# tc-mb/llama.cpp-omni

Measured on AMD Instinct MI355X. Metric: llama-bench tg128 tok/s (decode, batch 1), Qwen3-8B Q4_K_M, higher is better.
Workload: dtype q4_K/q6_K weights x q8_K activations (int8 dot, f32 accumulate); 1 GPU; Qwen3-8B Q4_K_M text-only decode, batch=1 per GPU, 1xMI355X (mul_mat_vec_q path); n_layer=36, n_embd=4096, n_ff=12288, n_vocab=151936, n_kv=2048, flash_attn=True, parallelism=replicas x1 (no collective)

## Files before the change

llama.cpp-omni_amd/csrc/kernels/mmv2.hip:

```cpp
#include "../kernels.hpp"
#include "mv_dev.hpp"
#include "mv2_dev.hpp"

namespace mi {

#ifndef MV2_BLOCK_LANE
#define MV2_BLOCK_LANE 1
#endif
#define MV2_WGT_PACKED 0x80000000u
static __device__ __forceinline__ int mv2_wgt_type(uint32_t wgt, int i) { const uint32_t c = (wgt >> (24 + 2 * i)) & 3u; return c == 1u ? GGML_TYPE_Q4_K : c == 2u ? GGML_TYPE_Q6_K : GGML_TYPE_Q8_0; }
typedef const __attribute__((address_space(4))) mv2_dev * mv2_karg;
#define MV2_REST_OFFSET 56
template <int TM, int NIT, bool PAIR, bool NT, int NW = MV2_WAVES, bool PARTS = false, int RWK = MV2_ROW_WAVES>
__global__ void __launch_bounds__(64 * NW) k_mv2(const char * W0, const float * x, const float * nw, const char * aux ,
                                                         uint32_t w_rs0, uint32_t qr0, uint32_t qr1, uint32_t qr2, float eps, uint32_t wgt , const mv2_dev rest) {
    __shared__ mv2_flags F;
    __shared__ double red[16];
    static_assert(!PARTS || (!PAIR && NIT == 1), "PARTS: one matrix of K = 4096 = n_head x 128 on the attention slices' partial states (x = the parts buffer)");
    constexpr int PBYTES = MV2_PARTS_NSL * 4096 * 4 + MV2_PARTS_NSL * 32 * 8;
    constexpr int XS = PARTS ? PBYTES + 512 - 32768 : 0;
    constexpr int RWN = PARTS ? MV2_PARTS_RW : RWK;
    static_assert(RWN <= NW - 1, "row waves are consumers");
    constexpr bool BL = MV2_BLOCK_LANE && (TM & 1) != 0 && TM != 4 + 1 && NIT == 1;
#ifndef MV2_HALF_BLOCK
#define MV2_HALF_BLOCK 1
#endif
    constexpr bool HBL = MV2_HALF_BLOCK && BL && !PAIR && TM == 1 && (NW == 10 || (MV2_HALF_BLOCK > 1 && NW == 9));
    constexpr int GRB = BL ? (PAIR || HBL ? 2 : 4) : 1;
    constexpr int C = NW - 1;
    constexpr int PW = 4 * NIT < C ? 4 * NIT : C;
    typedef mv2_geo<2304, 1, NIT, XS> geo0;
    MV2_STAMP_DECL;
    MV2_STAMP(0);
#ifdef MV2_TRACE
    tr_[6] = __builtin_amdgcn_s_getreg((4 ) | (0 << 6) | (31 << 11));
    if (threadIdx.x < 64) tr_[5] = __builtin_amdgcn_s_getreg((20 ) | (0 << 6) | (31 << 11));
#endif
    if (threadIdx.x < sizeof(mv2_flags) / 4) ((uint32_t *) &F)[threadIdx.x] = 0u;
    asm volatile("s_waitcnt lgkmcnt(0)\n\ts_barrier" ::: "memory");
    const int wiw = __builtin_amdgcn_readfirstlane(threadIdx.x >> 6);
    const int wg  = blockIdx.x;
#ifndef MV2_NO_STAGGER
    if (wiw == 0 || wiw >= NW - RWN) __builtin_amdgcn_s_setprio(3);
    else if (wiw <= PW) __builtin_amdgcn_s_sleep(12);
    else { __builtin_amdgcn_s_sleep(40); }
#endif
    uint64_t kp = (uint64_t) (uintptr_t) __builtin_amdgcn_kernarg_segment_ptr();
    asm volatile("" : "+s"(kp));
    const mv2_karg R = (mv2_karg) (uintptr_t) (kp + MV2_REST_OFFSET);
    (void) rest;
    const int K = 4096 * NIT;
    mv2_mat M;
    M.W = W0; M.w_rs = w_rs0; M.nrows = 0; M.q = (int) (qr0 & 0xffffu); M.r = (int) (qr0 >> 16); M.wg0 = 0; M.resid = PAIR ? nullptr : aux; M.dst = nullptr;
    M.type = TM == 2 ? GGML_TYPE_Q6_K : (TM == 4 ? GGML_TYPE_Q8_0 : (TM == 3 ? mv2_wgt_type(wgt, 0) : GGML_TYPE_Q4_K));
    int mi_ = 0;
    const int wg1 = (int) (wgt & 0xfffu);
    if (!PAIR && wg >= wg1) {
        const int wg2 = (int) ((wgt >> 12) & 0xfffu);
        mi_ = wg >= wg2 ? 2 : 1;
        if (wgt & MV2_WGT_PACKED) {
            const uint64_t offs = (uint64_t) (uintptr_t) aux;
            const int32_t off16 = (int32_t) (mi_ == 2 ? (uint32_t) (offs >> 32) : (uint32_t) offs);
            const uint32_t qr = mi_ == 2 ? qr2 : qr1;
            M.W = W0 + (int64_t) off16 * 16; M.q = (int) (qr & 0xffffu); M.r = (int) (qr >> 16); M.wg0 = mi_ == 2 ? wg2 : wg1; M.resid = nullptr;
            M.type = mv2_wgt_type(wgt, mi_);
            M.w_rs = (uint32_t) (K / 256) * (M.type == GGML_TYPE_Q4_K ? 144u : M.type == GGML_TYPE_Q6_K ? 210u : 272u);
        } else {
            const __attribute__((address_space(4))) uint32_t * wsrc = (const __attribute__((address_space(4))) uint32_t *) &R->m[mi_];
            uint32_t wbuf[sizeof(mv2_mat) / 4];
#pragma unroll
            for (size_t k = 0; k < sizeof(mv2_mat) / 4; ++k) wbuf[k] = wsrc[k];
            __builtin_memcpy(&M, wbuf, sizeof M);
        }
    }
    if (!PAIR && (wgt & MV2_WGT_PACKED)) M.resid = nullptr;
    const char * img = nullptr;
    if (x == nullptr) { asm volatile("" ::: "memory"); img = R->src.img; }
    const mv1_src src = { x, nw, eps, img };
    const char * W1 = aux;
    const int lw = wg - M.wg0;
    const int G0 = __builtin_amdgcn_readfirstlane(lw * M.q + (lw < M.r ? lw : M.r));
    const int ntask = __builtin_amdgcn_readfirstlane(M.q + (lw < M.r ? 1 : 0));
    char * im = mv1_lds;
    char * stg = mv1_lds + geo0::IMG;
    char * rstg = stg + geo0::STG;
    char * ringp = rstg + geo0::RSTG;
    constexpr bool Q80 = TM == 4;
    const bool q4 = TM == 1 || ((TM & 1) && M.type == GGML_TYPE_Q4_K);
    MV2_STAMP(1);
    if (wiw == 0) {
        const size_t wbytes = (size_t) (G0 + ntask) * M.w_rs;
        const mv1_rsrc rs0 = mv1_make_rsrc(M.W, wbytes), rs1 = mv1_make_rsrc(PAIR ? W1 : M.W, wbytes);
        if constexpr (Q80) mv2_loader<4352, PAIR ? 2 : 1, NIT, C, NT, XS, RWN>(rs0, rs1, (uint32_t) M.w_rs, G0, ntask * NIT, mv2_lds_addr(ringp), &F MV2_TR_ARG);
        else if (q4) mv2_loader<2304, PAIR ? 2 : 1, NIT, C, NT, XS, RWN, GRB>(rs0, rs1, (uint32_t) M.w_rs, G0, ntask * NIT, mv2_lds_addr(ringp), &F MV2_TR_ARG);
        else if constexpr ((TM & 2) != 0 && !PAIR) mv2_loader<3360, 1, NIT, C, NT, XS, RWN>(rs0, rs1, (uint32_t) M.w_rs, G0, ntask * NIT, mv2_lds_addr(ringp), &F MV2_TR_ARG);
        MV2_STAMP(7);
    } else {
        const int c = wiw - 1, lane = threadIdx.x & 63;
        const char * resid_p = PAIR ? nullptr : M.resid;
        if constexpr (PARTS) { if (c >= C - RWN) mv2_parts_loader((const char *) x, K, c - (C - RWN), resid_p, G0, ntask, mv2_lds_addr(stg), mv2_lds_addr(rstg), &F MV2_TR_ARG); }
        else if (c >= C - RWN) mv2_row_loader<RWN>(src, K, c - (C - RWN), resid_p, G0, ntask, mv2_lds_addr(stg), mv2_lds_addr(rstg), &F MV2_TR_ARG);
        uint32_t img_need = 4 * NIT;
        if constexpr (PARTS) { if (c < 4) mv2_prologue_parts<TM == 4>(K, c, im, stg, (float *) (stg + PBYTES), &F MV2_TR_ARG); }
        else if (src.img) { if constexpr (Q80) mv2_image_copy_q80<C>(src.img, K, c, im, &F); else mv2_image_copy<C>(src.img, K, c, im, &F); img_need = C; }
        else if (c < PW) mv2_prologue<NIT, Q80, PW, RWN>(src, K, c, im, stg, red, &F MV2_TR_ARG);
        { uint32_t spins = 0; while (mv2_peek(MV2_FLAG(F.img_cnt)) < img_need) { __builtin_amdgcn_s_sleep(4); if (++spins > MV2_SPIN_MAX) __builtin_trap(); } asm volatile("" ::: "memory"); }
        float resid = 0.0f;
        if (resid_p) { mv2_await(MV2_FLAG(F.x_landed), RWN); const int r = c + lane * C; if (r < ntask) resid = *(const float *) (rstg + r * 4); }
        MV2_STAMP(4);
        char * dst = R->m[mi_].dst;
        if constexpr (Q80) mv2_consume_q80<PAIR ? 2 : 1, NIT, C, PAIR, XS>(im, ringp, K, c, ntask, dst, G0 + c, resid, &F);
        else if (q4) {
            if constexpr (HBL) mv2_consume_q4k_h<NIT, C, XS>(im, ringp, K, c, ntask, dst, G0, rstg, resid_p != nullptr, &F);
            else if constexpr (BL) mv2_consume_q4k_b<NIT, C, PAIR, XS>(im, ringp, K, c, ntask, dst, G0, rstg, resid_p != nullptr, &F);
            else mv2_consume_q4k<PAIR ? 2 : 1, NIT, C, PAIR, XS>(im, ringp, K, c, ntask, dst, G0 + c, resid, &F);
        }
        else if constexpr ((TM & 2) != 0 && !PAIR) mv2_consume_q6k<NIT, C, XS>(im, ringp, K, c, ntask, dst, G0 + c, resid, &F);
        MV2_STAMP(7);
    }
    MV2_STAMP_FLUSH;
}

}

namespace mi {

static int mv2_dev_ordinal() { int dev = 0; HIP_CHECK(hipGetDevice(&dev)); return dev >= 0 && dev < 64 ? dev : 0; }
int mv2_cus_of(int dev) {
    static int n[64] = { 0 };
    if (dev < 0 || dev >= 64) dev = 0;
    if (!n[dev]) { hipDeviceProp_t p; HIP_CHECK(hipGetDeviceProperties(&p, dev)); n[dev] = p.multiProcessorCount > 0 ? p.multiProcessorCount : 256; }
    return n[dev];
}
int mv2_cus() { return mv2_cus_of(mv2_dev_ordinal()); }
static long g_mv2_launches = 0;
long mmv2_launches() { return g_mv2_launches; }

bool mmv2_ok(const mv1_args & a) {
    if (a.nmat < 1 || a.nmat > 3 || (a.K != 4096 && a.K != 12288)) return false;
    if (a.K == 12288 && a.norm_w && !a.img) return false;
    const bool q80 = a.m[0].type == GGML_TYPE_Q8_0;
    if (a.W_up && (a.nmat != 1 || (a.m[0].type != GGML_TYPE_Q4_K && !q80) || a.K != 4096 || a.m[0].resid || ((uintptr_t) a.W_up & 15) != 0)) return false;
    const int cus = mv2_cus();
    for (int i = 0; i < a.nmat; ++i) {
        const mmv_mat & m = a.m[i];
        if (q80 ? m.type != GGML_TYPE_Q8_0 : (m.type != GGML_TYPE_Q4_K && m.type != GGML_TYPE_Q6_K)) return false;
        if (m.nrows <= 0 || (uint64_t) m.nrows * m.w_rs > 0xffffffffull) return false;
        if (((uintptr_t) m.W & 15) != 0 || m.w_rs % 16 != 0) return false;
        if (((uintptr_t) m.dst & 3) != 0 || ((uintptr_t) m.resid & 3) != 0) return false;
        if (m.resid && m.nrows > (int64_t) cus * 256) return false;
    }
    if (a.parts)
        return a.nslice == MV2_PARTS_NSL && a.K == 4096 && a.nmat == 1 && !a.W_up && !a.norm_w && !a.img && !a.x && ((uintptr_t) a.parts & 15) == 0;
    if (a.img) return ((uintptr_t) a.img & 15) == 0;
    return a.x && ((uintptr_t) a.x & 15) == 0 && ((uintptr_t) a.norm_w & 15) == 0;
}

template <int TM, int NIT, bool PAIR, bool NT, int NW = MV2_WAVES, bool PARTS = false, int RWK = MV2_ROW_WAVES>
static void mv2_launch(const mv2_dev & d, int grid, hipStream_t st, const float * parts = nullptr) {
    const size_t lds = 160 * 1024 - 512;
    static bool attr[64] = { false };
    const int dev = mv2_dev_ordinal();
    if (!attr[dev]) { HIP_CHECK(hipFuncSetAttribute((const void *) k_mv2<TM, NIT, PAIR, NT, NW, PARTS, RWK>, hipFuncAttributeMaxDynamicSharedMemorySize, (int) lds)); attr[dev] = true; }
    static_assert(offsetof(mv2_dev, src) % 8 == 0, "argument block layout");
    auto qr = [&](int i) { return (uint32_t) d.m[i].q | ((uint32_t) d.m[i].r << 16); };
    auto tcode = [&](int i) { return d.m[i].type == GGML_TYPE_Q4_K ? 1u : d.m[i].type == GGML_TYPE_Q6_K ? 2u : 3u; };
    const int wg1 = d.nmat > 1 ? d.m[1].wg0 : grid, wg2 = d.nmat > 2 ? d.m[2].wg0 : grid;
    uint32_t wgt = (uint32_t) wg1 | ((uint32_t) wg2 << 12) | (tcode(0) << 24) | (tcode(d.nmat > 1 ? 1 : 0) << 26) | (tcode(d.nmat > 2 ? 2 : 0) << 28);
    const char * aux = PAIR ? d.W1 : d.m[0].resid;
    bool packed = !PAIR && d.nmat > 1 && grid < 4096;
    int64_t off[3] = { 0, 0, 0 };
    for (int i = 0; i < d.nmat && packed; ++i) {
        const uint32_t tight = (uint32_t) (d.K / 256) * (d.m[i].type == GGML_TYPE_Q4_K ? 144u : d.m[i].type == GGML_TYPE_Q6_K ? 210u : 272u);
        off[i] = ((int64_t) (intptr_t) d.m[i].W - (int64_t) (intptr_t) d.m[0].W) / 16;
        if (d.m[i].resid || d.m[i].q > 0xffff || d.m[i].r > 0xffff || (i > 0 && (d.m[i].w_rs != tight || off[i] != (int64_t) (int32_t) off[i] || (((intptr_t) d.m[i].W - (intptr_t) d.m[0].W) & 15) != 0))) packed = false;
    }
    if (packed) { wgt |= MV2_WGT_PACKED; aux = (const char *) (uintptr_t) ((uint64_t) (uint32_t) (int32_t) off[1] | ((uint64_t) (uint32_t) (int32_t) off[2] << 32)); }
    if (d.m[0].q > 0xffff || d.m[0].r > 0xffff || grid > 4095) { fprintf(stderr, "[mi355x] mmv2: %d rows per workgroup\n", d.m[0].q); abort(); }
    k_mv2<TM, NIT, PAIR, NT, NW, PARTS, RWK><<<dim3(grid), dim3(64 * NW), lds, st>>>(d.m[0].W, PARTS ? parts : (d.src.img ? nullptr : d.src.x), PARTS ? nullptr : d.src.nw, aux, d.m[0].w_rs, qr(0), qr(d.nmat > 1 ? 1 : 0), qr(d.nmat > 2 ? 2 : 0), d.src.eps, wgt, d);
}

#ifndef MV2_Q6_SHARE
#define MV2_Q6_SHARE 1.7
#endif
static int mv2_plan(const mv1_args & a, mv2_dev & d, int & tm) {
    const int cus = mv2_cus();
    double bytes[3], total = 0; int64_t tasks = 0; tm = 0;
    for (int i = 0; i < a.nmat; ++i) {
        bytes[i] = (double) a.m[i].nrows * (double) (a.m[i].type == GGML_TYPE_Q4_K ? 144 : a.m[i].type == GGML_TYPE_Q6_K ? 210 : 272) * (double) (a.K / 256);
#ifdef MV2_LAB_NW
        { static const double q6w = getenv("MV2_Q6_WEIGHT") ? atof(getenv("MV2_Q6_WEIGHT")) : MV2_Q6_SHARE; if (a.nmat > 1 && a.m[i].type == GGML_TYPE_Q6_K) bytes[i] *= q6w; }
#else
        if (a.nmat > 1 && a.m[i].type == GGML_TYPE_Q6_K) bytes[i] *= MV2_Q6_SHARE;
#endif
        total += bytes[i]; tasks += a.m[i].nrows;
        tm |= a.m[i].type == GGML_TYPE_Q4_K ? 1 : a.m[i].type == GGML_TYPE_Q6_K ? 2 : 4;
    }
    int grid = (int) (tasks < cus ? tasks : cus);
    if (grid < a.nmat) grid = a.nmat;
    d.nmat = a.nmat; d.K = (int) a.K; d.W1 = (const char *) a.W_up;
    d.src = { a.img ? nullptr : a.x, a.img ? nullptr : a.norm_w, a.eps, (const char *) a.img };
    int acc_w = 0; double acc_b = 0;
    for (int i = 0; i < 3; ++i) {
        if (i >= a.nmat) { d.m[i] = d.m[0]; d.m[i].wg0 = grid; continue; }
        acc_b += bytes[i];
        int end = i == a.nmat - 1 ? grid : (int) (grid * (acc_b / total) + 0.5);
        if (end <= acc_w) end = acc_w + 1;
        if (end > grid - (a.nmat - 1 - i)) end = grid - (a.nmat - 1 - i);
        const int nwg = end - acc_w;
        d.m[i] = { (const char *) a.m[i].W, (char *) a.m[i].dst, (const char *) a.m[i].resid, (uint32_t) a.m[i].w_rs, (int) a.m[i].nrows, a.m[i].type, acc_w, (int) (a.m[i].nrows / nwg), (int) (a.m[i].nrows % nwg) };
        acc_w = end;
    }
    return grid;
}

void mmv2(const mv1_args & a, hipStream_t st) {
    if (!mmv2_ok(a)) { fprintf(stderr, "[mi355x] mmv2: unsupported arguments (K=%lld)\n", (long long) a.K); abort(); }
    mv2_dev d; int tm;
    const int grid = mv2_plan(a, d, tm);
    ++g_mv2_launches;
    const bool pair = a.W_up != nullptr;
    static const bool nw16 = getenv("MI355X_MV2_NW16") != nullptr;
    const bool small = !nw16 && a.nmat == 1 && a.m[0].nrows <= 16384;
#ifdef MV2_LAB_NW
    {
        auto nw_env = [](const char * k, int dflt) { const char * e = getenv(k); return e ? atoi(e) : dflt; };
        static const int nw_pair = nw_env("MV2_NW_PAIR", 16), nw_grp = nw_env("MV2_NW_GRP", 12), nw_s4 = nw_env("MV2_NW_SMALL4", 10), nw_s12 = nw_env("MV2_NW_SMALL12", 10);
#define MV2_LAB_GO(TMv, NITv, PAIRv, nw) do { switch (nw) { case 9: mv2_launch<TMv, NITv, PAIRv, true, 9>(d, grid, st); break; case 10: mv2_launch<TMv, NITv, PAIRv, true, 10>(d, grid, st); break; \
        case 12: mv2_launch<TMv, NITv, PAIRv, true, 12>(d, grid, st); break; case 13: mv2_launch<TMv, NITv, PAIRv, true, 13>(d, grid, st); break; default: mv2_launch<TMv, NITv, PAIRv, true, 16>(d, grid, st); } return; } while (0)
        if (tm != 4 && !a.parts) {
            if (pair) MV2_LAB_GO(1, 1, true, nw_pair);
            if (a.K == 4096 && a.nmat > 1) { if (tm == 1) MV2_LAB_GO(1, 1, false, nw_grp); if (tm == 2) MV2_LAB_GO(2, 1, false, nw_grp); MV2_LAB_GO(3, 1, false, nw_grp); }
            if (a.K == 4096 && small) { if (tm == 1) MV2_LAB_GO(1, 1, false, nw_s4); MV2_LAB_GO(2, 1, false, nw_s4); }
            if (a.K == 12288 && small) { if (tm == 1) MV2_LAB_GO(1, 3, false, nw_s12); MV2_LAB_GO(2, 3, false, nw_s12); }
        }
    }
#endif
    if (tm == 4) {
        static const int q80_nw = getenv("MI355X_MV2_Q80_NW") ? atoi(getenv("MI355X_MV2_Q80_NW")) : -1;
        static const int q80_grp = getenv("MI355X_MV2_Q80_NW_GRP") ? atoi(getenv("MI355X_MV2_Q80_NW_GRP")) : -1;
        const int nwq = nw16 ? 16 : small ? (q80_nw > 0 ? q80_nw : 16) : (a.nmat > 1 && a.K == 4096) ? (q80_grp > 0 ? q80_grp : 10) : 16;
        if (pair)              mv2_launch<4, 1, true, true>(d, grid, st);
        else if (a.parts)      mv2_launch<4, 1, false, true, 10, true>(d, grid, st, a.parts);
        else if (a.K == 4096)  { if (nwq == 10) mv2_launch<4, 1, false, true, 10>(d, grid, st); else if (nwq == 12) mv2_launch<4, 1, false, true, 12>(d, grid, st); else mv2_launch<4, 1, false, true>(d, grid, st); }
        else                   { if (nwq == 10) mv2_launch<4, 3, false, true, 10>(d, grid, st); else if (nwq == 12) mv2_launch<4, 3, false, true, 12>(d, grid, st); else mv2_launch<4, 3, false, true>(d, grid, st); }
        return;
    }
    if (pair)               { mv2_launch<1, 1, true, true>(d, grid, st); return; }
    if (a.parts) {
        if (tm == 1) mv2_launch<1, 1, false, true, 10, true>(d, grid, st, a.parts);
        else         mv2_launch<2, 1, false, true, 10, true>(d, grid, st, a.parts);
        return;
    }
    if (a.K == 4096) {
        if (a.nmat > 1 && !nw16) {
            if (tm == 1)      mv2_launch<1, 1, false, true, 9>(d, grid, st);
            else if (tm == 2) mv2_launch<2, 1, false, true, 12>(d, grid, st);
            else              mv2_launch<3, 1, false, true, 9>(d, grid, st);
        } else if (small) {
            if (tm == 1)      mv2_launch<1, 1, false, true, 10>(d, grid, st);
            else              mv2_launch<2, 1, false, true, 10>(d, grid, st);
        } else {
            if (tm == 1)      mv2_launch<1, 1, false, true>(d, grid, st);
            else if (tm == 2 && a.nmat == 1 && !nw16) mv2_launch<2, 1, false, true, 9>(d, grid, st);
            else if (tm == 2) mv2_launch<2, 1, false, true>(d, grid, st);
            else              mv2_launch<3, 1, false, true>(d, grid, st);
        }
    } else {
        if (a.nmat > 1) {
            if (tm == 1)      mv2_launch<1, 3, false, true>(d, grid, st);
            else if (tm == 2) mv2_launch<2, 3, false, true>(d, grid, st);
            else              mv2_launch<3, 3, false, true>(d, grid, st);
        } else if (small) {
            if (tm == 1)      mv2_launch<1, 3, false, true, 10>(d, grid, st);
            else              mv2_launch<2, 3, false, true, 10>(d, grid, st);
        } else {
            if (tm == 1)      mv2_launch<1, 3, false, true>(d, grid, st);
            else              mv2_launch<2, 3, false, true>(d, grid, st);
        }
    }
}

}
```

llama.cpp-omni_amd/csrc/kernels/mv2_dev.hpp:

```cpp
#pragma once
#include "../kernels.hpp"
#include "mv_dev.hpp"

namespace mi {

typedef __attribute__((address_space(3))) void * mv2_lds_ptr;
static __device__ __forceinline__ uint32_t mv2_lds_addr(const void * p) { return (uint32_t) (uintptr_t) (mv2_lds_ptr) p; }

#ifdef MV2_TRACE
__device__ unsigned long long * mv2_trace_buf = nullptr;
#define MV2_STAMP_DECL uint32_t tr_[8] = { 0, 0, 0, 0, 0, 0, 0, 0 }
#define MV2_TR_PARAM , uint32_t (&tr_)[8]
#define MV2_TR_ARG , tr_
#define MV2_STAMP(i) do { tr_[i] = (uint32_t) __builtin_amdgcn_s_memrealtime(); asm volatile("" : "+s"(tr_[i]) :: "memory"); } while (0)
#define MV2_STAMP_FLUSH do { if (mv2_trace_buf) { const int l_ = threadIdx.x & 63; uint32_t v_ = 0; _Pragma("unroll") for (int i_ = 0; i_ < 8; ++i_) if (l_ == i_) v_ = tr_[i_]; \
    if (l_ < 8) mv2_trace_buf[(size_t) (blockIdx.x * (blockDim.x >> 6) + (threadIdx.x >> 6)) * 8 + l_] = v_; } } while (0)
#else
#define MV2_STAMP_DECL
#define MV2_TR_PARAM
#define MV2_TR_ARG
#define MV2_STAMP(i) do { } while (0)
#define MV2_STAMP_FLUSH do { } while (0)
#endif

#define MV2_LGKM0()   asm volatile("s_waitcnt lgkmcnt(0)" ::: "memory")
template <int N> static __device__ __forceinline__ void mv2_vmcnt() { static_assert(N >= 0 && N < 64, "vmcnt is 6 bits"); asm volatile("s_waitcnt vmcnt(%0)" :: "n"(N) : "memory"); }

#ifndef MV2_WAVES
#define MV2_WAVES 16
#endif
#ifndef MV2_ROW_WAVES
#define MV2_ROW_WAVES 4
#endif

struct mv2_mat { const char * W; char * dst; const char * resid; uint32_t w_rs; int nrows; int type; int wg0; int q; int r; };
struct mv2_dev { mv2_mat m[3]; int nmat; const char * W1; mv1_src src; int K; };

struct mv2_flags {
    uint32_t landed;
    uint32_t rows_issued;
    uint32_t x_landed;
    uint32_t rows_landed;
    uint32_t sum_cnt, img_cnt;
    uint32_t scale_ready; float scale;
    uint32_t consumed[16];
};
typedef __attribute__((address_space(3))) uint32_t mv2_lds_u32;
#define MV2_FLAG(x) ((mv2_lds_u32 *) &(x))
static __device__ __forceinline__ uint32_t mv2_peek(const mv2_lds_u32 * p) { const uint32_t v = *(const volatile mv2_lds_u32 *) p; return __builtin_amdgcn_readfirstlane(v); }
static __device__ __forceinline__ void mv2_poke(mv2_lds_u32 * p, uint32_t v) { if ((threadIdx.x & 63) == 0) *(volatile mv2_lds_u32 *) p = v; }
static __device__ __forceinline__ void mv2_arrive(mv2_lds_u32 * p) {
    asm volatile("" ::: "memory");
    if ((threadIdx.x & 63) == 0) __hip_atomic_fetch_add(p, 1u, __ATOMIC_RELAXED, __HIP_MEMORY_SCOPE_WORKGROUP);
    asm volatile("" ::: "memory");
}
#ifndef MV2_SPIN_MAX
#if defined(MV2_TRACE) || defined(MV2_DEBUG)
#define MV2_SPIN_MAX (1u << 21)
#else
#define MV2_SPIN_MAX (1u << 28)
#endif
#endif
#ifndef MV2_SLEEP
#define MV2_SLEEP 1
#endif
static __device__ __forceinline__ void mv2_await(const mv2_lds_u32 * p, uint32_t n) {
    uint32_t spins = 0;
    while (mv2_peek(p) < n) { __builtin_amdgcn_s_sleep(1); if (++spins > MV2_SPIN_MAX) __builtin_trap(); }
    asm volatile("" ::: "memory");
}

static __device__ __forceinline__ void mv2_lane_map(int lane, int & blk, int & q) {
    const int l5 = lane & 31;
    const bool ga = l5 < 4 || (l5 >= 12 && l5 < 16) || (l5 >= 20 && l5 < 28);
    blk = ga ? (l5 < 4 ? l5 : (l5 < 16 ? l5 - 8 : l5 - 12)) : (l5 < 12 ? l5 - 4 : (l5 < 20 ? l5 - 8 : l5 - 16));
    q = (ga ? 0 : 1) + 2 * (lane >> 5);
}

template <int PIECE, bool NT>
static __device__ __forceinline__ void mv2_dma_piece(const mv1_rsrc rs, uint32_t soff, uint32_t lds, uint32_t v16, uint32_t v4) {
    static_assert(PIECE == 2304 || PIECE == 3360 || PIECE == 4352, "16 Q4_K / Q6_K super-blocks, or 128 Q8_0 blocks");
    if constexpr (PIECE == 4352) {
        if constexpr (NT)
            asm volatile("s_mov_b32 m0, %0\n\ts_nop 0\n\t"
                         "buffer_load_dwordx4 %1, %3, %4 offen nt lds\n\t"
                         "buffer_load_dwordx4 %1, %3, %4 offen offset:1024 nt lds\n\t"
                         "buffer_load_dwordx4 %1, %3, %4 offen offset:2048 nt lds\n\t"
                         "buffer_load_dwordx4 %1, %3, %4 offen offset:3072 nt lds\n\t"
                         "s_mov_b32 m0, %6\n\ts_nop 0\n\t"
                         "buffer_load_dword %2, %3, %5 offen nt lds"
                         :: "s"(lds), "v"(v16), "v"(v4), "s"(rs), "s"(soff), "s"(soff + 4096u), "s"(lds + 4096u) : "memory", "m0");
        else
            asm volatile("s_mov_b32 m0, %0\n\ts_nop 0\n\t"
                         "buffer_load_dwordx4 %1, %3, %4 offen lds\n\t"
                         "buffer_load_dwordx4 %1, %3, %4 offen offset:1024 lds\n\t"
                         "buffer_load_dwordx4 %1, %3, %4 offen offset:2048 lds\n\t"
                         "buffer_load_dwordx4 %1, %3, %4 offen offset:3072 lds\n\t"
                         "s_mov_b32 m0, %6\n\ts_nop 0\n\t"
                         "buffer_load_dword %2, %3, %5 offen lds"
                         :: "s"(lds), "v"(v16), "v"(v4), "s"(rs), "s"(soff), "s"(soff + 4096u), "s"(lds + 4096u) : "memory", "m0");
    } else if constexpr (PIECE == 2304) {
        if constexpr (NT)
            asm volatile("s_mov_b32 m0, %0\n\ts_nop 0\n\t"
                         "buffer_load_dwordx4 %1, %3, %4 offen nt lds\n\t"
                         "buffer_load_dwordx4 %1, %3, %4 offen offset:1024 nt lds\n\t"
                         "buffer_load_dword %2, %3, %4 offen offset:2048 nt lds"
                         :: "s"(lds), "v"(v16), "v"(v4), "s"(rs), "s"(soff) : "memory", "m0");
        else
            asm volatile("s_mov_b32 m0, %0\n\ts_nop 0\n\t"
                         "buffer_load_dwordx4 %1, %3, %4 offen lds\n\t"
                         "buffer_load_dwordx4 %1, %3, %4 offen offset:1024 lds\n\t"
                         "buffer_load_dword %2, %3, %4 offen offset:2048 lds"
                         :: "s"(lds), "v"(v16), "v"(v4), "s"(rs), "s"(soff) : "memory", "m0");
    } else {
        uint64_t keep;
        if constexpr (NT)
            asm volatile("s_mov_b32 m0, %1\n\ts_nop 0\n\t"
                         "buffer_load_dwordx4 %2, %3, %4 offen nt lds\n\t"
                         "buffer_load_dwordx4 %2, %3, %4 offen offset:1024 nt lds\n\t"
                         "buffer_load_dwordx4 %2, %3, %4 offen offset:2048 nt lds\n\t"
                         "s_mov_b64 %0, exec\n\ts_mov_b64 exec, 0x3ffff\n\t"
                         "buffer_load_dwordx4 %2, %3, %4 offen offset:3072 nt lds\n\t"
                         "s_mov_b64 exec, %0"
                         : "=&s"(keep) : "s"(lds), "v"(v16), "s"(rs), "s"(soff) : "memory", "m0");
        else
            asm volatile("s_mov_b32 m0, %1\n\ts_nop 0\n\t"
                         "buffer_load_dwordx4 %2, %3, %4 offen lds\n\t"
                         "buffer_load_dwordx4 %2, %3, %4 offen offset:1024 lds\n\t"
                         "buffer_load_dwordx4 %2, %3, %4 offen offset:2048 lds\n\t"
                         "s_mov_b64 %0, exec\n\ts_mov_b64 exec, 0x3ffff\n\t"
                         "buffer_load_dwordx4 %2, %3, %4 offen offset:3072 lds\n\t"
                         "s_mov_b64 exec, %0"
                         : "=&s"(keep) : "s"(lds), "v"(v16), "s"(rs), "s"(soff) : "memory", "m0");
        (void) v4;
    }
}

template <int PIECE, int R, int NIT, int XS = 0> struct mv2_geo {
    static constexpr int VM    = (PIECE == 2304 ? 3 : PIECE == 3360 ? 4 : 5) * R;
    static constexpr int D     = 60 / VM;
    static constexpr int B     = R == 2 ? 2 : 4;
    static constexpr int SLOTB = PIECE * R;
    static constexpr int IMG   = NIT * 16 * 324 + 16;
    static constexpr int STG   = (NIT == 1 ? 32768 : 49152) + XS;
    static constexpr int RSTG  = 1024;
    static constexpr int NS    = (160 * 1024 - 512 - IMG - STG - RSTG) / SLOTB;
    static_assert(NS >= D + NIT + B, "ring too small");
};

template <int VM, int K_> struct mv2_drain {
    static __device__ __forceinline__ void go(int n, mv2_lds_u32 * landed) {
        if (n > K_) { mv2_vmcnt<VM * K_>(); mv2_poke(landed, (uint32_t) (n - K_)); }
        if constexpr (K_ > 0) mv2_drain<VM, K_ - 1>::go(n, landed);
    }
};
template <int PIECE, int R, int NIT, int C, bool NT, int XS = 0, int RWN = MV2_ROW_WAVES, int GR = 1>
static __device__ __forceinline__ void mv2_loader(const mv1_rsrc rs0, const mv1_rsrc rs1, uint32_t rs32, int G0, int T, uint32_t ring, mv2_flags * F MV2_TR_PARAM) {
    typedef mv2_geo<PIECE, R, NIT, XS> geo;
    constexpr int VM = geo::VM, D = geo::D, B = geo::B, SLOTB = geo::SLOTB, NS = geo::NS;
    const int lane = threadIdx.x & 63;
    const uint32_t v16 = 16u * (uint32_t) lane, v4 = 4u * (uint32_t) lane;
    uint32_t so = __builtin_amdgcn_readfirstlane((uint32_t) G0 * rs32);
    const uint32_t row_skip = __builtin_amdgcn_readfirstlane(rs32 - (uint32_t) (NIT * PIECE));
    uint32_t la = __builtin_amdgcn_readfirstlane(ring);
    const uint32_t ring_end = __builtin_amdgcn_readfirstlane(ring + (uint32_t) (NS * SLOTB));
    int it = 0;
    auto issue = [&]() {
#pragma unroll
        for (int r = 0; r < R; ++r) mv2_dma_piece<PIECE, NT>(r == 1 ? rs1 : rs0, so, la + (uint32_t) (r * PIECE), v16, v4);
        so += (uint32_t) PIECE; la += (uint32_t) SLOTB;
        if (la == ring_end) la = __builtin_amdgcn_readfirstlane(ring);
        if (NIT > 1) { if (++it == NIT) { it = 0; so += row_skip; } } else so += row_skip;
    };
    int n = 0, free_tasks = 0;
#ifndef MV2_PRE
#define MV2_PRE 0
#endif
    for (; n < MV2_PRE && n < T; ++n) issue();
#ifndef MV2_PAIR_WAITS
    if (R != 2)
#endif
    mv2_await(MV2_FLAG(F->rows_issued), RWN);
    MV2_STAMP(2);
    while (n < T) {
        const int nb_ = T - n < B ? T - n : B;
        const int last = n + nb_ - 1;
        if (last >= NS) {
            const int need = (last - NS) / NIT + 1;
            uint32_t spins = 0;
            while (free_tasks < need) {
                uint32_t k = lane < C ? (uint32_t) lane + *(const volatile mv2_lds_u32 *) MV2_FLAG(F->consumed[lane & 15]) * (uint32_t) C : 0xffffffffu;
                { const uint32_t o = (uint32_t) __builtin_amdgcn_update_dpp(-1, (int) k, 0xB1, 0xf, 0xf, false);  k = __builtin_elementwise_min(k, o); }
                { const uint32_t o = (uint32_t) __builtin_amdgcn_update_dpp(-1, (int) k, 0x4E, 0xf, 0xf, false);  k = __builtin_elementwise_min(k, o); }
                { const uint32_t o = (uint32_t) __builtin_amdgcn_update_dpp(-1, (int) k, 0x141, 0xf, 0xf, false); k = __builtin_elementwise_min(k, o); }
                { const uint32_t o = (uint32_t) __builtin_amdgcn_update_dpp(-1, (int) k, 0x140, 0xf, 0xf, false); k = __builtin_elementwise_min(k, o); }
                free_tasks = (int) __builtin_amdgcn_readfirstlane(k) * GR;
                if (free_tasks < need) { __builtin_amdgcn_s_sleep(1); if (++spins > MV2_SPIN_MAX) __builtin_trap(); }
            }
            asm volatile("" ::: "memory");
        }
#pragma unroll
        for (int i = 0; i < B; ++i) if (i < nb_) issue();
        n += nb_;
        if (n > D - B) { mv2_vmcnt<VM * (D - B)>(); mv2_poke(MV2_FLAG(F->landed), (uint32_t) (n - (D - B))); }
    }
    mv2_drain<VM, D - B - 1>::go(n, MV2_FLAG(F->landed));
}

template <int RWN = MV2_ROW_WAVES>
static __device__ __forceinline__ void mv2_row_loader(const mv1_src src, int K, int rw, const char * resid, int G0, int ntask, uint32_t stg, uint32_t rstg, mv2_flags * F MV2_TR_PARAM) {
    const int lane = threadIdx.x & 63;
    const uint32_t v16 = 16u * (uint32_t) lane, v4 = 4u * (uint32_t) lane;
#ifdef MV2_ROWSTART
    mv2_arrive(MV2_FLAG(F->rows_issued));
#endif
    const int nb = K >> 8;
    if (!src.img) {
        const __amdgpu_buffer_rsrc_t xr = __builtin_amdgcn_make_buffer_rsrc((void *) src.x, (short) 0, K * 4, 0x00020000);
        MV2_STAMP(2);
        for (int b = rw, i = 0; b < nb; b += RWN, ++i) {
            if (i == 1) MV2_STAMP(3);
            asm volatile("s_mov_b32 m0, %0\n\ts_nop 0\n\tbuffer_load_dwordx4 %1, %2, %3 offen lds" :: "s"(__builtin_amdgcn_readfirstlane(stg + (uint32_t) b * 1024u)), "v"(v16), "s"(xr), "s"(__builtin_amdgcn_readfirstlane((uint32_t) b * 1024u)) : "memory", "m0");
        }
    }
    if (resid && rw == 0) {
        const __amdgpu_buffer_rsrc_t rr = __builtin_amdgcn_make_buffer_rsrc((void *) (resid + (size_t) G0 * 4), (short) 0, ntask * 4, 0x00020000);
        for (int b = 0; b * 64 < ntask; ++b)
            asm volatile("s_mov_b32 m0, %0\n\ts_nop 0\n\tbuffer_load_dword %1, %2, %3 offen lds" :: "s"(__builtin_amdgcn_readfirstlane(rstg + (uint32_t) b * 256u)), "v"(v4), "s"(rr), "s"(__builtin_amdgcn_readfirstlane((uint32_t) b * 256u)) : "memory", "m0");
    }
    MV2_STAMP(5);
    mv2_arrive(MV2_FLAG(F->rows_issued));
    if (!src.img && src.nw) {
        const __amdgpu_buffer_rsrc_t wr = __builtin_amdgcn_make_buffer_rsrc((void *) src.nw, (short) 0, K * 4, 0x00020000);
        static_assert(16 % RWN == 0, "norm weights of K = 4096: 16 pieces over the row waves");
#pragma unroll
        for (int i = 0; i < 16 / RWN; ++i) {
            const int b = rw + i * RWN;
            asm volatile("s_mov_b32 m0, %0\n\ts_nop 0\n\tbuffer_load_dwordx4 %1, %2, %3 offen lds" :: "s"(__builtin_amdgcn_readfirstlane(stg + (uint32_t) (K * 4) + (uint32_t) b * 1024u)), "v"(v16), "s"(wr), "s"(__builtin_amdgcn_readfirstlane((uint32_t) b * 1024u)) : "memory", "m0");
        }
        mv2_vmcnt<16 / RWN>();
        mv2_arrive(MV2_FLAG(F->x_landed));
    } else {
        mv2_vmcnt<0>();
        mv2_arrive(MV2_FLAG(F->x_landed));
    }
    mv2_vmcnt<0>();
    mv2_arrive(MV2_FLAG(F->rows_landed));
}

template <int CTRL> static __device__ __forceinline__ uint32_t mv2_dpp_row(uint32_t v) { return (uint32_t) __builtin_amdgcn_update_dpp(0, (int) v, CTRL, 0xf, 0xf, true); }
static __device__ __forceinline__ void mv2_q8k_rows(const f32x4 (&y)[4], int lane, int b, int nb, char * im) {
    const int i = lane & 15;
    uint32_t key = 0;
#pragma unroll
    for (int m = 0; m < 4; ++m)
#pragma unroll
        for (int e = 0; e < 4; ++e) { const uint32_t u = __float_as_uint(y[m][e]); key = umax32(key, __builtin_amdgcn_alignbit(u, u, 31)); }
    key = umax32(key, mv2_dpp_row<0xB1>(key));
    key = umax32(key, mv2_dpp_row<0x4E>(key));
    key = umax32(key, mv2_dpp_row<0x141>(key));
    key = umax32(key, mv2_dpp_row<0x140>(key));
    const bool zero = (key >> 1) == 0u;
    const float mval = __uint_as_float(__builtin_amdgcn_alignbit(key, key, 1));
    const float iscale = zero ? 0.0f : -127.0f / mval;
    char * qs = im + b * 272;
    int16_t * bs32 = (int16_t *) (im + mv1_img_bs(nb)) + b * 8;
    int16_t * b16  = (int16_t *) (im + mv1_img_b16(nb)) + b * 16;
#pragma unroll
    for (int m = 0; m < 4; ++m) {
        uint32_t t[4];
#pragma unroll
        for (int e = 0; e < 4; ++e) { const float p = iscale * y[m][e]; t[e] = __float_as_uint(p + 12582912.0f); }
        const uint32_t lo = __builtin_amdgcn_perm(t[1], t[0], 0x0c0c0400u), hi = __builtin_amdgcn_perm(t[3], t[2], 0x04000c0cu);
        const uint32_t qd = lo | hi;
        *(uint32_t *) (qs + 64 * m + 4 * i) = qd;
        int s = dot4(qd, 0x01010101u, 0);
        s += (int) mv2_dpp_row<0xB1>((uint32_t) s);
        s += (int) mv2_dpp_row<0x4E>((uint32_t) s);
        if ((i & 3) == 0) b16[mv1_b16_pos(4 * m + (i >> 2))] = (int16_t) s;
        s += (int) mv2_dpp_row<0x141>((uint32_t) s);
        if ((i & 7) == 0) bs32[2 * m + (i >> 3)] = (int16_t) s;
    }
    if (i == 0) *((float *) (im + mv1_img_d(nb)) + b) = zero ? 0.0f : 1.0f / iscale;
}

static __device__ __forceinline__ void mv2_q80_rows(const f32x4 (&y)[4], int lane, int b, int K, char * im) {
    const int i = lane & 15;
#pragma unroll
    for (int m = 0; m < 4; ++m) {
        float amax = fmaxf(fmaxf(fabsf(y[m][0]), fabsf(y[m][1])), fmaxf(fabsf(y[m][2]), fabsf(y[m][3])));
        amax = fmaxf(amax, __uint_as_float(mv2_dpp_row<0xB1>(__float_as_uint(amax))));
        amax = fmaxf(amax, __uint_as_float(mv2_dpp_row<0x4E>(__float_as_uint(amax))));
        amax = fmaxf(amax, __uint_as_float(mv2_dpp_row<0x141>(__float_as_uint(amax))));
        const float d = amax / 127.0f;
        const float id = amax != 0.0f ? 127.0f / amax : 0.0f;
        uint32_t qd = 0;
#pragma unroll
        for (int e = 0; e < 4; ++e) qd |= ((uint32_t) (int) __builtin_rintf(y[m][e] * id) & 0xffu) << (8 * e);
        *(uint32_t *) (im + 256 * b + 64 * m + 4 * i) = qd;
        if ((i & 7) == 0) *(float *) (im + K + (8 * b + 2 * m + (i >> 3)) * 4) = h2f(f2h(d));
    }
}

template <int NIT, bool Q80 = false, int PW = 4 * NIT, int RWN = MV2_ROW_WAVES>
static __device__ __forceinline__ void mv2_prologue(const mv1_src s, int K, int pw, char * im, const char * stg, double * red, mv2_flags * F MV2_TR_PARAM) {
    const int lane = threadIdx.x & 63, row = lane >> 4, i = lane & 15, nb = K >> 8;
    constexpr int NG = (4 * NIT + PW - 1) / PW;
    mv2_await(MV2_FLAG(F->x_landed), RWN);
    MV2_STAMP(2);
    float scale = 1.0f;
    f32x4 x[NG][4];
    if (s.nw) {
        bool last = false;
#pragma unroll
        for (int g = 0; g < NG; ++g) {
            const int mw = pw + g * PW;
            if (mw >= 4 * NIT) break;
            const char * xp = stg + (mw * 4 + row) * 1024 + 16 * i;
#pragma unroll
            for (int m = 0; m < 4; ++m) x[g][m] = *(const f32x4 *) (xp + 256 * m);
            double ss = 0.0;
#pragma unroll
            for (int m = 0; m < 4; ++m)
#pragma unroll
                for (int e = 0; e < 4; ++e) ss += (double) (x[g][m][e] * x[g][m][e]);
            ss = wave_sum_f64(ss);
            if (lane == 0) red[mw] = ss;
            asm volatile("" ::: "memory");
            uint32_t prev = 0;
            if (lane == 0) prev = __hip_atomic_fetch_add(MV2_FLAG(F->sum_cnt), 1u, __ATOMIC_RELAXED, __HIP_MEMORY_SCOPE_WORKGROUP);
            prev = __builtin_amdgcn_readfirstlane(prev);
            asm volatile("" ::: "memory");
            if (prev == (uint32_t) (4 * NIT - 1)) last = true;
        }
        if (last) {
            double tot = 0.0;
#pragma unroll
            for (int w = 0; w < 4 * NIT; ++w) tot += *(const volatile double *) &red[w];
            const float mean = (float) ((K & (K - 1)) == 0 ? tot * (1.0 / (double) K) : tot / (double) K);
            const float sc = 1.0f / sqrtf(mean + s.eps);
            if (lane == 0) *(volatile __attribute__((address_space(3))) float *) &F->scale = sc;
            mv2_poke(MV2_FLAG(F->scale_ready), 1u);
            scale = sc;
        } else {
            mv2_await(MV2_FLAG(F->scale_ready), 1u);
            scale = *(const volatile __attribute__((address_space(3))) float *) &F->scale;
        }
    }
    MV2_STAMP(3);
    if (s.nw) mv2_await(MV2_FLAG(F->rows_landed), RWN);
#pragma unroll
    for (int g = 0; g < NG; ++g) {
        const int mw = pw + g * PW;
        if (mw >= 4 * NIT) break;
        const int b = mw * 4 + row;
        f32x4 y[4];
        if (s.nw) {
            const char * wp = stg + K * 4 + b * 1024 + 16 * i;
#pragma unroll
            for (int m = 0; m < 4; ++m) {
                const f32x4 w = *(const f32x4 *) (wp + 256 * m);
#pragma unroll
                for (int e = 0; e < 4; ++e) y[m][e] = (x[g][m][e] * scale) * w[e];
            }
        } else {
            const char * xp = stg + b * 1024 + 16 * i;
#pragma unroll
            for (int m = 0; m < 4; ++m) y[m] = *(const f32x4 *) (xp + 256 * m);
        }
        if constexpr (Q80) mv2_q80_rows(y, lane, b, K, im); else mv2_q8k_rows(y, lane, b, nb, im);
        mv2_arrive(MV2_FLAG(F->img_cnt));
    }
    MV2_STAMP(5);
}
#define MV2_PARTS_NSL 4
#define MV2_PARTS_RW  8
static __device__ __forceinline__ void mv2_parts_loader(const char * parts, int K, int rw, const char * resid, int G0, int ntask, uint32_t stg, uint32_t rstg, mv2_flags * F MV2_TR_PARAM) {
    const int lane = threadIdx.x & 63;
    const uint32_t v16 = 16u * (uint32_t) lane, v4 = 4u * (uint32_t) lane;
    const int bytes = MV2_PARTS_NSL * K * 4 + MV2_PARTS_NSL * (K / 128) * 8, np = (bytes + 1023) >> 10;
    const __amdgpu_buffer_rsrc_t xr = __builtin_amdgcn_make_buffer_rsrc((void *) parts, (short) 0, bytes, 0x00020000);
    MV2_STAMP(2);
    for (int b = rw, i = 0; b < np; b += MV2_PARTS_RW, ++i) {
        if (i == 1) MV2_STAMP(3);
        asm volatile("s_mov_b32 m0, %0\n\ts_nop 0\n\tbuffer_load_dwordx4 %1, %2, %3 offen lds" :: "s"(__builtin_amdgcn_readfirstlane(stg + (uint32_t) b * 1024u)), "v"(v16), "s"(xr), "s"(__builtin_amdgcn_readfirstlane((uint32_t) b * 1024u)) : "memory", "m0");
    }
    if (resid && rw == 0) {
        const __amdgpu_buffer_rsrc_t rr = __builtin_amdgcn_make_buffer_rsrc((void *) (resid + (size_t) G0 * 4), (short) 0, ntask * 4, 0x00020000);
        for (int b = 0; b * 64 < ntask; ++b)
            asm volatile("s_mov_b32 m0, %0\n\ts_nop 0\n\tbuffer_load_dword %1, %2, %3 offen lds" :: "s"(__builtin_amdgcn_readfirstlane(rstg + (uint32_t) b * 256u)), "v"(v4), "s"(rr), "s"(__builtin_amdgcn_readfirstlane((uint32_t) b * 256u)) : "memory", "m0");
    }
    MV2_STAMP(5);
    mv2_arrive(MV2_FLAG(F->rows_issued));
    mv2_vmcnt<0>();
    mv2_arrive(MV2_FLAG(F->x_landed));
    mv2_arrive(MV2_FLAG(F->rows_landed));
}
template <bool Q80 = false>
static __device__ __forceinline__ void mv2_prologue_parts(int K, int pw, char * im, const char * stg, float * coef , mv2_flags * F MV2_TR_PARAM) {
    const int lane = threadIdx.x & 63, row = lane >> 4, i = lane & 15, nb = K >> 8, nh = K >> 7;
    constexpr int NSL = MV2_PARTS_NSL;
    mv2_await(MV2_FLAG(F->x_landed), MV2_PARTS_RW);
    MV2_STAMP(2);
    const int b = pw * 4 + row;
    {
        const int h = 2 * b + ((i >> 2) & 1), sl = i & 3;
        const u32x2 ms = *(const u32x2 *) (stg + (size_t) NSL * K * 4 + ((size_t) sl * nh + h) * 8);
        const float Ms = __uint_as_float(ms[0]), Ss = __uint_as_float(ms[1]);
        float M = fmaxf(Ms, __uint_as_float(mv2_dpp_row<0xB1>(__float_as_uint(Ms))));
        M = fmaxf(M, __uint_as_float(mv2_dpp_row<0x4E>(__float_as_uint(M))));
        const float f = Ms == -INFINITY ? 0.0f : expf(Ms - M);
        float den = Ss * f;
        den += __uint_as_float(mv2_dpp_row<0xB1>(__float_as_uint(den)));
        den += __uint_as_float(mv2_dpp_row<0x4E>(__float_as_uint(den)));
        const float cf = den == 0.0f ? 0.0f : f * (1.0f / den);
        if (i < 8) coef[b * 8 + i] = cf;
    }
    asm volatile("" ::: "memory");
    const f32x4 c0 = *(const f32x4 *) (coef + b * 8), c1 = *(const f32x4 *) (coef + b * 8 + 4);
    f32x4 y[4];
    const char * xp = stg + b * 1024 + 16 * i;
#pragma unroll
    for (int m = 0; m < 4; ++m) {
        const f32x4 cc = m < 2 ? c0 : c1;
        f32x4 acc = { 0.0f, 0.0f, 0.0f, 0.0f };
#pragma unroll
        for (int sl = 0; sl < NSL; ++sl) {
            const f32x4 o = *(const f32x4 *) (xp + (size_t) sl * K * 4 + 256 * m);
#pragma unroll
            for (int e = 0; e < 4; ++e) acc[e] = fmaf(cc[sl], o[e], acc[e]);
        }
        y[m] = acc;
    }
    MV2_STAMP(3);
    if constexpr (Q80) mv2_q80_rows(y, lane, b, K, im); else mv2_q8k_rows(y, lane, b, nb, im);
    mv2_arrive(MV2_FLAG(F->img_cnt));
    MV2_STAMP(5);
}

template <int C>
static __device__ __forceinline__ void mv2_image_copy_q80(const char * img, int K, int c, char * im, mv2_flags * F) {
    const int lane = threadIdx.x & 63;
    for (int i = c * 64 + lane; i < (K + K / 8) / 16; i += 64 * C) ((u32x4 *) im)[i] = ((const u32x4 *) img)[i];
    mv2_arrive(MV2_FLAG(F->img_cnt));
}
template <int C>
static __device__ __forceinline__ void mv2_image_copy(const char * img, int K, int c, char * im, mv2_flags * F) {
    const int lane = threadIdx.x & 63, nb = K >> 8;
    for (int i = c * 64 + lane; i < nb * 16; i += 64 * C) *(u32x4 *) (im + (i >> 4) * 272 + (i & 15) * 16) = ((const u32x4 *) img)[i];
    for (int i = c * 64 + lane; i < nb * 8; i += 64 * C) {
        const uint32_t p = *(const uint32_t *) (img + K + i * 4);
        *(int16_t *) (im + mv1_img_bs(nb) + i * 2) = (int16_t) ((int) (int16_t) (p & 0xffff) + (int) (int16_t) (p >> 16));
        const int b = i >> 3, s0 = (i & 7) * 2;
        *(int16_t *) (im + mv1_img_b16(nb) + b * 32 + mv1_b16_pos(s0) * 2)     = (int16_t) (p & 0xffff);
        *(int16_t *) (im + mv1_img_b16(nb) + b * 32 + mv1_b16_pos(s0 + 1) * 2) = (int16_t) (p >> 16);
    }
    for (int i = c * 64 + lane; i < nb; i += 64 * C) *(float *) (im + mv1_img_d(nb) + i * 4) = *(const float *) (img + K + (K >> 3) + i * 4);
    mv2_arrive(MV2_FLAG(F->img_cnt));
}

static __device__ __forceinline__ void mv2_wait_step(int t, uint32_t & seen, mv2_flags * F) {
    uint32_t spins = 0;
    while (seen <= (uint32_t) t) { seen = mv2_peek(MV2_FLAG(F->landed)); if (seen <= (uint32_t) t) { __builtin_amdgcn_s_sleep(MV2_SLEEP); if (++spins > MV2_SPIN_MAX) __builtin_trap(); } }
    asm volatile("" ::: "memory");
}

struct mv2_out { float res; int nres, k0; };
template <int C>
static __device__ __forceinline__ void mv2_out_flush(mv2_out & o, char * dst, int row0, float resid) {
    const int lane = threadIdx.x & 63;
    if (lane < o.nres) *(float *) (dst + (size_t) (row0 + (o.k0 + lane) * C) * 4) = o.res + resid;
    o.k0 += o.nres; o.nres = 0;
}

struct mv2_q4k_act { u32x4 a[4]; uint32_t bsw; float yd; };
static __device__ __forceinline__ void mv2_q4k_dot(const u32x4 H, const u32x4 Q, const u32x4 P, const mv2_q4k_act & A, uint32_t sel, float & acc, float & accm) {
    const uint32_t s_lo = H[1] & 0x3f3f3f3fu, s_hi = (H[3] & 0x0f0f0f0fu) | ((H[1] >> 2) & 0x30303030u);
    const uint32_t m_lo = H[2] & 0x3f3f3f3fu, m_hi = ((H[3] >> 4) & 0x0f0f0f0fu) | ((H[2] >> 2) & 0x30303030u);
    const uint32_t sw = __builtin_amdgcn_perm(s_hi, s_lo, sel), mw = __builtin_amdgcn_perm(m_hi, m_lo, sel);
    const int sc0 = sw & 0xff, sc1 = sw >> 8;
    const int mn0 = mw & 0xff, mn1 = mw >> 8;
    const float dx = h2f((uint16_t) (H[0] & 0xffff)), dmin = h2f((uint16_t) (H[0] >> 16));
    const int bs0 = (int) (int16_t) (A.bsw & 0xffff), bs1 = (int) (int16_t) (A.bsw >> 16);
    int dl = 0, dh = 0;
#pragma unroll
    for (int k = 0; k < 4; ++k) {
        dl = dot4(Q[k] & 0x0f0f0f0fu, A.a[0][k], dl); dh = dot4((Q[k] >> 4) & 0x0f0f0f0fu, A.a[2][k], dh);
        dl = dot4(P[k] & 0x0f0f0f0fu, A.a[1][k], dl); dh = dot4((P[k] >> 4) & 0x0f0f0f0fu, A.a[3][k], dh);
    }
    const int isum = mad24(sc0, dl, mul24(sc1, dh));
    const int msum = mad24(mn0, bs0, mul24(mn1, bs1));
    acc  = fmaf(dx * A.yd, (float) isum, acc);
    accm = fmaf(dmin * A.yd, (float) msum, accm);
}
static __device__ __forceinline__ void mv2_q4k_act_load(const char * im, int nb, int ib, int q, mv2_q4k_act & A) {
    const char * la = im + ib * 272 + 64 * q;
#pragma unroll
    for (int k = 0; k < 4; ++k) A.a[k] = *(const u32x4 *) (la + 16 * k);
    A.bsw = *(const uint32_t *) (im + mv1_img_bs(nb) + ib * 16 + 4 * q);
    A.yd  = *(const float *) (im + mv1_img_d(nb) + ib * 4);
}
static __device__ __forceinline__ uint32_t mv2_q4k_sel(int q) { return 0x0c0c0000u | (uint32_t) ((q < 2 ? 0 : 4) + 2 * (q & 1)) | ((uint32_t) ((q < 2 ? 0 : 4) + 2 * (q & 1) + 1) << 8); }
template <int R, int NIT, int C, bool PAIR, int XS = 0>
static __device__ __forceinline__ void mv2_consume_q4k(const char * im, const char * ringp, int K, int c, int ntask, char * dst, int row0, float resid, mv2_flags * F) {
    typedef mv2_geo<2304, R, NIT, XS> geo;
    constexpr int SLOTB = geo::SLOTB, NS = geo::NS;
    const int lane = threadIdx.x & 63, nb = K >> 8;
    int blk, q; mv2_lane_map(lane, blk, q);
    const uint32_t sel = mv2_q4k_sel(q);
    mv2_q4k_act A[NIT];
#pragma unroll
    for (int it = 0; it < NIT; ++it) mv2_q4k_act_load(im, nb, it * 16 + blk, q, A[it]);
    const char * wl = ringp + blk * 144;
    uint32_t seen = 0;
    mv2_out o = { 0.0f, 0, 0 };
    int k = 0;
    for (int j = c; j < ntask; j += C, ++k) {
        float acc[R], accm[R];
#pragma unroll
        for (int r = 0; r < R; ++r) { acc[r] = 0.0f; accm[r] = 0.0f; }
#pragma unroll
        for (int it = 0; it < NIT; ++it) {
            const int t = __builtin_amdgcn_readfirstlane(j * NIT + it);
            mv2_wait_step(t, seen, F);
            const char * p = wl + (t % NS) * SLOTB;
            u32x4 H[R], Q[R], P[R];
#pragma unroll
            for (int r = 0; r < R; ++r) { H[r] = *(const u32x4 *) (p + r * 2304); Q[r] = *(const u32x4 *) (p + r * 2304 + 16 + 32 * q); P[r] = *(const u32x4 *) (p + r * 2304 + 32 + 32 * q); }
            if (it == NIT - 1) { MV2_LGKM0(); mv2_poke(MV2_FLAG(F->consumed[c]), (uint32_t) (k + 1)); }
#pragma unroll
            for (int r = 0; r < R; ++r) mv2_q4k_dot(H[r], Q[r], P[r], A[it], sel, acc[r], accm[r]);
        }
        if (PAIR) {
            const float gsum = wave_sum_f32(acc[0] - accm[0]), usum = wave_sum_f32(acc[R - 1] - accm[R - 1]);
            if (lane == o.nres) o.res = mv1_silu(gsum) * usum;
        } else {
            const float s = wave_sum_f32(acc[0] - accm[0]);
            if (lane == o.nres) o.res = s;
        }
        if (++o.nres == 64) mv2_out_flush<C>(o, dst, row0, resid);
    }
    mv2_out_flush<C>(o, dst, row0, resid);
}

template <int NIT, int C, bool PAIR, int XS = 0>
static __device__ __forceinline__ void mv2_consume_q4k_b(const char * im, const char * ringp, int K, int c, int ntask, char * dst, int G0, const char * rstg, bool has_resid, mv2_flags * F) {
    constexpr int R = PAIR ? 2 : 1, GR = PAIR ? 2 : 4;
    typedef mv2_geo<2304, R, NIT, XS> geo;
    constexpr int SLOTB = geo::SLOTB, NS = geo::NS;
    const int lane = threadIdx.x & 63, nb = K >> 8;
    const int blk = lane & 15, r = PAIR ? lane >> 5 : lane >> 4, mat = PAIR ? (lane >> 4) & 1 : 0;
    const int ng = (ntask + GR - 1) / GR;
    uint32_t seen = 0;
    int k = 0;
    for (int g = c; g < ng; g += C, ++k) {
        const int j = g * GR + r;
        const bool valid = j < ntask;
        const int jl = (g * GR + GR <= ntask ? g * GR + GR : ntask) - 1;
        float accv = 0.0f, accm = 0.0f;
#pragma unroll
        for (int it = 0; it < NIT; ++it) {
            mv2_wait_step(__builtin_amdgcn_readfirstlane(jl * NIT + it), seen, F);
            const int t = (valid ? j : jl) * NIT + it;
            const int b0 = __builtin_amdgcn_readfirstlane((g * GR * NIT + it) % NS);
            int slot = b0 + (t - (g * GR * NIT + it));
            if (slot >= NS) slot -= NS;
            const char * p = ringp + slot * SLOTB + mat * 2304 + blk * 144;
            const u32x4 H = *(const u32x4 *) p;
            u32x4 Q[8];
#pragma unroll
            for (int e = 0; e < 8; ++e) Q[e] = *(const u32x4 *) (p + 16 + 16 * e);
            const int ib = it * 16 + blk;
            const char * la = im + ib * 272;
            const u32x4 bsv = *(const u32x4 *) (im + mv1_img_bs(nb) + ib * 16);
            const float yd = *(const float *) (im + mv1_img_d(nb) + ib * 4);
            if (it == NIT - 1) { MV2_LGKM0(); mv2_poke(MV2_FLAG(F->consumed[c]), (uint32_t) (k + 1)); }
            const uint32_t s_lo = H[1] & 0x3f3f3f3fu, s_hi = (H[3] & 0x0f0f0f0fu) | ((H[1] >> 2) & 0x30303030u);
            const uint32_t m_lo = H[2] & 0x3f3f3f3fu, m_hi = ((H[3] >> 4) & 0x0f0f0f0fu) | ((H[2] >> 2) & 0x30303030u);
            int isum = 0, msum = 0;
#pragma unroll
            for (int jg = 0; jg < 4; ++jg) {
                const u32x4 a0 = *(const u32x4 *) (la + 64 * jg), a1 = *(const u32x4 *) (la + 64 * jg + 16), a2 = *(const u32x4 *) (la + 64 * jg + 32), a3 = *(const u32x4 *) (la + 64 * jg + 48);
                int dl = 0, dh = 0;
#pragma unroll
                for (int e = 0; e < 4; ++e) {
                    dl = dot4(Q[2 * jg][e] & 0x0f0f0f0fu, a0[e], dl); dh = dot4((Q[2 * jg][e] >> 4) & 0x0f0f0f0fu, a2[e], dh);
                    dl = dot4(Q[2 * jg + 1][e] & 0x0f0f0f0fu, a1[e], dl); dh = dot4((Q[2 * jg + 1][e] >> 4) & 0x0f0f0f0fu, a3[e], dh);
                }
                const uint32_t sw = jg < 2 ? s_lo : s_hi, mw = jg < 2 ? m_lo : m_hi;
                const int sh = 16 * (jg & 1);
                const int sc0 = (int) ((sw >> sh) & 0xffu), sc1 = (int) ((sw >> (sh + 8)) & 0xffu), mn0 = (int) ((mw >> sh) & 0xffu), mn1 = (int) ((mw >> (sh + 8)) & 0xffu);
                const uint32_t bw = bsv[jg];
                isum = mad24(sc0, dl, mad24(sc1, dh, isum));
                msum = mad24(mn0, (int) (int16_t) (bw & 0xffff), mad24(mn1, (int) (int16_t) (bw >> 16), msum));
            }
            const float dx = h2f((uint16_t) (H[0] & 0xffff)), dmin = h2f((uint16_t) (H[0] >> 16));
            accv = fmaf(dx * yd, (float) isum, accv);
            accm = fmaf(dmin * yd, (float) msum, accm);
        }
        float v = accv - accm;
        v += __uint_as_float(mv2_dpp_row<0xB1>(__float_as_uint(v))); v += __uint_as_float(mv2_dpp_row<0x4E>(__float_as_uint(v)));
        v += __uint_as_float(mv2_dpp_row<0x141>(__float_as_uint(v))); v += __uint_as_float(mv2_dpp_row<0x140>(__float_as_uint(v)));
        if constexpr (PAIR) {
            const float o = __shfl_xor(v, 16, 64);
            if (valid && mat == 0 && blk == 0) *(float *) (dst + (size_t) (G0 + j) * 4) = mv1_silu(v) * o;
        } else {
            if (valid && blk == 0) *(float *) (dst + (size_t) (G0 + j) * 4) = v + (has_resid ? *(const float *) (rstg + j * 4) : 0.0f);
        }
    }
}

template <int NIT, int C, int XS = 0>
static __device__ __forceinline__ void mv2_consume_q4k_h(const char * im, const char * ringp, int K, int c, int ntask, char * dst, int G0, const char * rstg, bool has_resid, mv2_flags * F) {
    constexpr int GR = 2;
    typedef mv2_geo<2304, 1, NIT, XS> geo;
    constexpr int SLOTB = geo::SLOTB, NS = geo::NS;
    const int lane = threadIdx.x & 63, nb = K >> 8;
    const int blk = lane & 15, h = (lane >> 4) & 1, r = lane >> 5;
    const int ng = (ntask + GR - 1) / GR;
    uint32_t seen = 0;
    int k = 0;
    for (int g = c; g < ng; g += C, ++k) {
        const int j = g * GR + r;
        const bool valid = j < ntask;
        const int jl = (g * GR + GR <= ntask ? g * GR + GR : ntask) - 1;
        float accv = 0.0f, accm = 0.0f;
#pragma unroll
        for (int it = 0; it < NIT; ++it) {
            mv2_wait_step(__builtin_amdgcn_readfirstlane(jl * NIT + it), seen, F);
            const int t = (valid ? j : jl) * NIT + it;
            const int b0 = __builtin_amdgcn_readfirstlane((g * GR * NIT + it) % NS);
            int slot = b0 + (t - (g * GR * NIT + it));
            if (slot >= NS) slot -= NS;
            const char * p = ringp + slot * SLOTB + blk * 144;
            const u32x4 H = *(const u32x4 *) p;
            u32x4 Q[4];
#pragma unroll
            for (int e = 0; e < 4; ++e) Q[e] = *(const u32x4 *) (p + 16 + 64 * h + 16 * e);
            const int ib = it * 16 + blk;
            const char * la = im + ib * 272 + 128 * h;
            u32x4 a[8];
#pragma unroll
            for (int e = 0; e < 8; ++e) a[e] = *(const u32x4 *) (la + 16 * e);
            const u32x2 bsv = *(const u32x2 *) (im + mv1_img_bs(nb) + ib * 16 + 8 * h);
            const float yd = *(const float *) (im + mv1_img_d(nb) + ib * 4);
            if (it == NIT - 1) { MV2_LGKM0(); mv2_poke(MV2_FLAG(F->consumed[c]), (uint32_t) (k + 1)); }
            const uint32_t sw = h ? ((H[3] & 0x0f0f0f0fu) | ((H[1] >> 2) & 0x30303030u)) : (H[1] & 0x3f3f3f3fu);
            const uint32_t mw = h ? (((H[3] >> 4) & 0x0f0f0f0fu) | ((H[2] >> 2) & 0x30303030u)) : (H[2] & 0x3f3f3f3fu);
            int isum = 0, msum = 0;
#pragma unroll
            for (int tj = 0; tj < 2; ++tj) {
                int dl = 0, dh = 0;
#pragma unroll
                for (int e = 0; e < 4; ++e) {
                    dl = dot4(Q[2 * tj][e] & 0x0f0f0f0fu, a[4 * tj][e], dl);         dh = dot4((Q[2 * tj][e] >> 4) & 0x0f0f0f0fu, a[4 * tj + 2][e], dh);
                    dl = dot4(Q[2 * tj + 1][e] & 0x0f0f0f0fu, a[4 * tj + 1][e], dl); dh = dot4((Q[2 * tj + 1][e] >> 4) & 0x0f0f0f0fu, a[4 * tj + 3][e], dh);
                }
                const int sh = 16 * tj;
                const int sc0 = (int) ((sw >> sh) & 0xffu), sc1 = (int) ((sw >> (sh + 8)) & 0xffu), mn0 = (int) ((mw >> sh) & 0xffu), mn1 = (int) ((mw >> (sh + 8)) & 0xffu);
                const uint32_t bw = bsv[tj];
                isum = mad24(sc0, dl, mad24(sc1, dh, isum));
                msum = mad24(mn0, (int) (int16_t) (bw & 0xffff), mad24(mn1, (int) (int16_t) (bw >> 16), msum));
            }
            const float dx = h2f((uint16_t) (H[0] & 0xffff)), dmin = h2f((uint16_t) (H[0] >> 16));
            accv = fmaf(dx * yd, (float) isum, accv);
            accm = fmaf(dmin * yd, (float) msum, accm);
        }
        float v = accv - accm;
        v += __uint_as_float(mv2_dpp_row<0xB1>(__float_as_uint(v))); v += __uint_as_float(mv2_dpp_row<0x4E>(__float_as_uint(v)));
        v += __uint_as_float(mv2_dpp_row<0x141>(__float_as_uint(v))); v += __uint_as_float(mv2_dpp_row<0x140>(__float_as_uint(v)));
        { const auto sw2 = __builtin_amdgcn_permlane16_swap(__float_as_uint(v), __float_as_uint(v), false, false); v = __uint_as_float((uint32_t) sw2[0]) + __uint_as_float((uint32_t) sw2[1]); }
        if (valid && blk == 0 && h == 0) *(float *) (dst + (size_t) (G0 + j) * 4) = v + (has_resid ? *(const float *) (rstg + j * 4) : 0.0f);
    }
}

typedef u32x4 __attribute__((aligned(2))) mv2_u32x4_a2;
typedef u32x2 __attribute__((aligned(2))) mv2_u32x2_a2;
struct mv2_q6k_act { u32x4 a[4]; u32x2 bq; float yd; };
struct mv2_q6k_lane { int blk, n, hf, qoff, hoff, soff; uint32_t sh, sel; };
static __device__ __forceinline__ mv2_q6k_lane mv2_q6k_lane_of(int lane) {
    mv2_q6k_lane L;
    L.blk = lane >> 2; L.n = (lane >> 1) & 1; L.hf = lane & 1;
    L.sel = (uint32_t) L.hf | ((uint32_t) (L.hf + 2) << 8) | ((uint32_t) (4 + L.hf) << 16) | ((uint32_t) (6 + L.hf) << 24);
    const int qraw = L.blk * 210 + 64 * L.n + 16 * L.hf;
    L.qoff = (qraw & ~3) - L.blk * 210; L.hoff = 128 + 32 * L.n - 64 * L.n; L.soff = 192 + 8 * L.n - 64 * L.n - 16 * L.hf;
    L.sh = (qraw & 2) ? 16u : 0u;
    return L;
}
static __device__ __forceinline__ void mv2_q6k_act_load(const char * im, int nb, int ib, const mv2_q6k_lane & L, mv2_q6k_act & A) {
    const char * la = im + ib * 272 + 128 * L.n + 16 * L.hf;
#pragma unroll
    for (int m = 0; m < 4; ++m) A.a[m] = *(const u32x4 *) (la + 32 * m);
    A.bq = *(const u32x2 *) (im + mv1_img_b16(nb) + ib * 32 + (8 * L.n + 4 * L.hf) * 2);
    A.yd = *(const float *) (im + mv1_img_d(nb) + ib * 4);
}
struct mv2_q6k_regs { u32x4 qla, qlb, qh; u32x2 sc; uint16_t dw; };
static __device__ __forceinline__ void mv2_q6k_read(const char * p, const mv2_q6k_lane & L, mv2_q6k_regs & Rg) {
    const __attribute__((address_space(3))) char * pa = (const __attribute__((address_space(3))) char *) (p + L.qoff);
    uint32_t d0[5], d1[5], d2[5], d3[3];
#pragma unroll
    for (int e = 0; e < 5; ++e) { d0[e] = *(const volatile mv2_lds_u32 *) (pa + 4 * e); d1[e] = *(const volatile mv2_lds_u32 *) (pa + 32 + 4 * e); d2[e] = *(const volatile mv2_lds_u32 *) (pa + L.hoff + 4 * e); }
#pragma unroll
    for (int e = 0; e < 3; ++e) d3[e] = *(const volatile mv2_lds_u32 *) (pa + L.soff + 4 * e);
#pragma unroll
    for (int e = 0; e < 4; ++e) { Rg.qla[e] = __builtin_amdgcn_alignbit(d0[e + 1], d0[e], L.sh); Rg.qlb[e] = __builtin_amdgcn_alignbit(d1[e + 1], d1[e], L.sh); Rg.qh[e] = __builtin_amdgcn_alignbit(d2[e + 1], d2[e], L.sh); }
    Rg.sc[0] = __builtin_amdgcn_alignbit(d3[1], d3[0], L.sh); Rg.sc[1] = __builtin_amdgcn_alignbit(d3[2], d3[1], L.sh);
    Rg.dw = *(const uint16_t *) (p + 208);
}
static __device__ __forceinline__ float mv2_q6k_dot(const mv2_q6k_regs & Rg, const mv2_q6k_act & A, uint32_t sel, float acc) {
    const uint32_t scw = __builtin_amdgcn_perm(Rg.sc[1], Rg.sc[0], sel);
    const int bs[4] = { (int) (int16_t) (A.bq[0] & 0xffff), (int) (int16_t) (A.bq[0] >> 16), (int) (int16_t) (A.bq[1] & 0xffff), (int) (int16_t) (A.bq[1] >> 16) };
    int d[4] = { 0, 0, 0, 0 };
#pragma unroll
    for (int e = 0; e < 4; ++e) {
        const uint32_t Aq = Rg.qla[e], Bq = Rg.qlb[e], Hq = Rg.qh[e];
        d[0] = dot4((Aq & 0x0f0f0f0fu)        | ((Hq << 4) & 0x30303030u), A.a[0][e], d[0]);
        d[1] = dot4((Bq & 0x0f0f0f0fu)        | ((Hq << 2) & 0x30303030u), A.a[1][e], d[1]);
        d[2] = dot4(((Aq >> 4) & 0x0f0f0f0fu) | (Hq & 0x30303030u),        A.a[2][e], d[2]);
        d[3] = dot4(((Bq >> 4) & 0x0f0f0f0fu) | ((Hq >> 2) & 0x30303030u), A.a[3][e], d[3]);
    }
    int isum = 0;
#pragma unroll
    for (int m = 0; m < 4; ++m) {
        const int scm = (int) (int8_t) ((scw >> (8 * m)) & 0xff);
        isum = mad24(scm, mad24(bs[m], -32, d[m]), isum);
    }
    return fmaf(h2f(Rg.dw) * A.yd, (float) isum, acc);
}
template <int NIT, int C, int XS = 0>
static __device__ __forceinline__ void mv2_consume_q6k(const char * im, const char * ringp, int K, int c, int ntask, char * dst, int row0, float resid, mv2_flags * F) {
    typedef mv2_geo<3360, 1, NIT, XS> geo;
    constexpr int SLOTB = geo::SLOTB, NS = geo::NS;
    const int lane = threadIdx.x & 63, nb = K >> 8;
    const mv2_q6k_lane L = mv2_q6k_lane_of(lane);
    mv2_q6k_act A[NIT];
#pragma unroll
    for (int it = 0; it < NIT; ++it) mv2_q6k_act_load(im, nb, it * 16 + L.blk, L, A[it]);
    const char * wl = ringp + L.blk * 210;
    uint32_t seen = 0;
    mv2_out o = { 0.0f, 0, 0 };
    int k = 0;
    for (int j = c; j < ntask; j += C, ++k) {
        float acc = 0.0f;
#pragma unroll
        for (int it = 0; it < NIT; ++it) {
            const int t = __builtin_amdgcn_readfirstlane(j * NIT + it);
            mv2_wait_step(t, seen, F);
            mv2_q6k_regs Rg;
            mv2_q6k_read(wl + (t % NS) * SLOTB, L, Rg);
            if (it == NIT - 1) { MV2_LGKM0(); mv2_poke(MV2_FLAG(F->consumed[c]), (uint32_t) (k + 1)); }
            acc = mv2_q6k_dot(Rg, A[it], L.sel, acc);
        }
        const float s = wave_sum_f32(acc);
        if (lane == o.nres) o.res = s;
        if (++o.nres == 64) mv2_out_flush<C>(o, dst, row0, resid);
    }
    mv2_out_flush<C>(o, dst, row0, resid);
}

struct mv2_q80_act { u32x4 a[4]; float yd[2]; };
static __device__ __forceinline__ void mv2_q80_act_load(const char * im, int K, int ib0 , mv2_q80_act & A) {
#pragma unroll
    for (int k = 0; k < 4; ++k) A.a[k] = *(const u32x4 *) (im + ib0 * 32 + 16 * k);
    A.yd[0] = *(const float *) (im + K + ib0 * 4); A.yd[1] = *(const float *) (im + K + ib0 * 4 + 4);
}
static __device__ __forceinline__ float mv2_q80_dot(const uint32_t (&w)[17], const mv2_q80_act & A, float acc) {
    int s0 = 0, s1 = 0;
#pragma unroll
    for (int e = 0; e < 8; ++e) {
        s0 = dot4(__builtin_amdgcn_alignbit(w[e + 1], w[e], 16), A.a[e >> 2][e & 3], s0);
        s1 = dot4(w[9 + e], A.a[2 + (e >> 2)][e & 3], s1);
    }
    acc = fmaf((float) s0, h2f((uint16_t) (w[0] & 0xffff)) * A.yd[0], acc);
    acc = fmaf((float) s1, h2f((uint16_t) (w[8] >> 16)) * A.yd[1], acc);
    return acc;
}
template <int R, int NIT, int C, bool PAIR, int XS = 0>
static __device__ __forceinline__ void mv2_consume_q80(const char * im, const char * ringp, int K, int c, int ntask, char * dst, int row0, float resid, mv2_flags * F) {
    typedef mv2_geo<4352, R, NIT, XS> geo;
    constexpr int SLOTB = geo::SLOTB, NS = geo::NS;
    const int lane = threadIdx.x & 63;
    mv2_q80_act A[NIT];
#pragma unroll
    for (int it = 0; it < NIT; ++it) mv2_q80_act_load(im, K, it * 128 + 2 * lane, A[it]);
    const __attribute__((address_space(3))) char * wl = (const __attribute__((address_space(3))) char *) (ringp + lane * 68);
    uint32_t seen = 0;
    mv2_out o = { 0.0f, 0, 0 };
    int k = 0;
    for (int j = c; j < ntask; j += C, ++k) {
        float acc[R];
#pragma unroll
        for (int r = 0; r < R; ++r) acc[r] = 0.0f;
#pragma unroll
        for (int it = 0; it < NIT; ++it) {
            const int t = __builtin_amdgcn_readfirstlane(j * NIT + it);
            mv2_wait_step(t, seen, F);
            const __attribute__((address_space(3))) char * p = wl + (t % NS) * SLOTB;
            uint32_t w[R][17];
#pragma unroll
            for (int r = 0; r < R; ++r)
#pragma unroll
                for (int e = 0; e < 17; ++e) w[r][e] = *(const volatile mv2_lds_u32 *) (p + r * 4352 + 4 * e);
            if (it == NIT - 1) { MV2_LGKM0(); mv2_poke(MV2_FLAG(F->consumed[c]), (uint32_t) (k + 1)); }
#pragma unroll
            for (int r = 0; r < R; ++r) acc[r] = mv2_q80_dot(w[r], A[it], acc[r]);
        }
        if (PAIR) {
            const float gsum = wave_sum_f32(acc[0]), usum = wave_sum_f32(acc[R - 1]);
            if (lane == o.nres) o.res = mv1_silu(gsum) * usum;
        } else {
            const float s = wave_sum_f32(acc[0]);
            if (lane == o.nres) o.res = s;
        }
        if (++o.nres == 64) mv2_out_flush<C>(o, dst, row0, resid);
    }
    mv2_out_flush<C>(o, dst, row0, resid);
}

}
```

Before: 613.6 tok/s.

## Prefetch and unpack first weight task before waiting on activation image

Consumer waves now read and unpack their first weight block from the LDS ring (nibble masking, scale and min extraction) before waiting for the activation image and residual to be ready. The gate wait is wrapped in a lambda and called after that early work, and the consumer index order is reversed so that consumers whose work becomes ready later are mapped differently. The aim is to hide weight decode latency behind the prologue that quantizes the activations. In exchange, the pinned, pre-unpacked weights raise VGPR pressure, and the reversed mapping changes which rows each wave handles.

```diff
diff --git a/llama.cpp-omni_amd/csrc/kernels/mmv2.hip b/llama.cpp-omni_amd/csrc/kernels/mmv2.hip
--- a/llama.cpp-omni_amd/csrc/kernels/mmv2.hip
+++ b/llama.cpp-omni_amd/csrc/kernels/mmv2.hip
@@ -6,6 +6,9 @@
 
 #ifndef MV2_BLOCK_LANE
 #define MV2_BLOCK_LANE 1
+#endif
+#ifndef MV2_PREPARE
+#define MV2_PREPARE 1
 #endif
 #define MV2_WGT_PACKED 0x80000000u
 static __device__ __forceinline__ int mv2_wgt_type(uint32_t wgt, int i) { const uint32_t c = (wgt >> (24 + 2 * i)) & 3u; return c == 1u ? GGML_TYPE_Q4_K : c == 2u ? GGML_TYPE_Q6_K : GGML_TYPE_Q8_0; }
@@ -28,6 +31,7 @@
     constexpr bool HBL = MV2_HALF_BLOCK && BL && !PAIR && TM == 1 && (NW == 10 || (MV2_HALF_BLOCK > 1 && NW == 9));
     constexpr int GRB = BL ? (PAIR || HBL ? 2 : 4) : 1;
     constexpr int C = NW - 1;
+    constexpr bool PREP = MV2_PREPARE > 1 ? (TM != 4) : (MV2_PREPARE == 1 && (TM & 1) != 0 && TM != 4 + 1 && NIT == 1 && !PAIR && !PARTS && NW == 9);
     constexpr int PW = 4 * NIT < C ? 4 * NIT : C;
     typedef mv2_geo<2304, 1, NIT, XS> geo0;
     MV2_STAMP_DECL;
@@ -97,6 +101,9 @@
         MV2_STAMP(7);
     } else {
         const int c = wiw - 1, lane = threadIdx.x & 63;
+#ifdef MV2_TRACE
+        tr_[6] = 0;
+#endif
         const char * resid_p = PAIR ? nullptr : M.resid;
         if constexpr (PARTS) { if (c >= C - RWN) mv2_parts_loader((const char *) x, K, c - (C - RWN), resid_p, G0, ntask, mv2_lds_addr(stg), mv2_lds_addr(rstg), &F MV2_TR_ARG); }
         else if (c >= C - RWN) mv2_row_loader<RWN>(src, K, c - (C - RWN), resid_p, G0, ntask, mv2_lds_addr(stg), mv2_lds_addr(rstg), &F MV2_TR_ARG);
@@ -104,18 +111,23 @@
         if constexpr (PARTS) { if (c < 4) mv2_prologue_parts<TM == 4>(K, c, im, stg, (float *) (stg + PBYTES), &F MV2_TR_ARG); }
         else if (src.img) { if constexpr (Q80) mv2_image_copy_q80<C>(src.img, K, c, im, &F); else mv2_image_copy<C>(src.img, K, c, im, &F); img_need = C; }
         else if (c < PW) mv2_prologue<NIT, Q80, PW, RWN>(src, K, c, im, stg, red, &F MV2_TR_ARG);
-        { uint32_t spins = 0; while (mv2_peek(MV2_FLAG(F.img_cnt)) < img_need) { __builtin_amdgcn_s_sleep(4); if (++spins > MV2_SPIN_MAX) __builtin_trap(); } asm volatile("" ::: "memory"); }
-        float resid = 0.0f;
-        if (resid_p) { mv2_await(MV2_FLAG(F.x_landed), RWN); const int r = c + lane * C; if (r < ntask) resid = *(const float *) (rstg + r * 4); }
-        MV2_STAMP(4);
+        const int lc = PREP ? C - 1 - c : c;
+        auto gate = [&]() -> float {
+            MV2_STAMP(6);
+            { uint32_t spins = 0; while (mv2_peek(MV2_FLAG(F.img_cnt)) < img_need) { __builtin_amdgcn_s_sleep(PREP ? 1 : 4); if (++spins > MV2_SPIN_MAX) __builtin_trap(); } asm volatile("" ::: "memory"); }
+            float resid = 0.0f;
+            if (resid_p) { mv2_await(MV2_FLAG(F.x_landed), RWN); const int r = lc + lane * C; if (r < ntask) resid = *(const float *) (rstg + r * 4); }
+            MV2_STAMP(4);
+            return resid;
+        };
         char * dst = R->m[mi_].dst;
-        if constexpr (Q80) mv2_consume_q80<PAIR ? 2 : 1, NIT, C, PAIR, XS>(im, ringp, K, c, ntask, dst, G0 + c, resid, &F);
+        if constexpr (Q80) { const float resid = gate(); mv2_consume_q80<PAIR ? 2 : 1, NIT, C, PAIR, XS>(im, ringp, K, lc, ntask, dst, G0 + lc, resid, &F); }
         else if (q4) {
-            if constexpr (HBL) mv2_consume_q4k_h<NIT, C, XS>(im, ringp, K, c, ntask, dst, G0, rstg, resid_p != nullptr, &F);
-            else if constexpr (BL) mv2_consume_q4k_b<NIT, C, PAIR, XS>(im, ringp, K, c, ntask, dst, G0, rstg, resid_p != nullptr, &F);
-            else mv2_consume_q4k<PAIR ? 2 : 1, NIT, C, PAIR, XS>(im, ringp, K, c, ntask, dst, G0 + c, resid, &F);
-        }
-        else if constexpr ((TM & 2) != 0 && !PAIR) mv2_consume_q6k<NIT, C, XS>(im, ringp, K, c, ntask, dst, G0 + c, resid, &F);
+            if constexpr (HBL) mv2_consume_q4k_h<NIT, C, XS, PREP>(im, ringp, K, lc, ntask, dst, G0, rstg, resid_p != nullptr, &F, gate);
+            else if constexpr (BL) mv2_consume_q4k_b<NIT, C, PAIR, XS, PREP>(im, ringp, K, lc, ntask, dst, G0, rstg, resid_p != nullptr, &F, gate);
+            else mv2_consume_q4k<PAIR ? 2 : 1, NIT, C, PAIR, XS, PREP>(im, ringp, K, lc, ntask, dst, G0 + lc, &F, gate);
+        }
+        else if constexpr ((TM & 2) != 0 && !PAIR) mv2_consume_q6k<NIT, C, XS, PREP>(im, ringp, K, lc, ntask, dst, G0 + lc, &F, gate);
         MV2_STAMP(7);
     }
     MV2_STAMP_FLUSH;
diff --git a/llama.cpp-omni_amd/csrc/kernels/mv2_dev.hpp b/llama.cpp-omni_amd/csrc/kernels/mv2_dev.hpp
--- a/llama.cpp-omni_amd/csrc/kernels/mv2_dev.hpp
+++ b/llama.cpp-omni_amd/csrc/kernels/mv2_dev.hpp
@@ -32,6 +32,16 @@
 #ifndef MV2_ROW_WAVES
 #define MV2_ROW_WAVES 4
 #endif
+#ifndef MV2_PREPARE
+#define MV2_PREPARE 1
+#endif
+static __device__ __forceinline__ void mv2_pin(uint32_t & v) { asm volatile("" : "+v"(v)); }
+static __device__ __forceinline__ void mv2_pin(int & v) { asm volatile("" : "+v"(v)); }
+static __device__ __forceinline__ void mv2_pin(float & v) { asm volatile("" : "+v"(v)); }
+static __device__ __forceinline__ void mv2_pin(u32x4 & v) {
+#pragma unroll
+    for (int e = 0; e < 4; ++e) { uint32_t t = v[e]; mv2_pin(t); v[e] = t; }
+}
 
 struct mv2_mat { const char * W; char * dst; const char * resid; uint32_t w_rs; int nrows; int type; int wg0; int q; int r; };
 struct mv2_dev { mv2_mat m[3]; int nmat; const char * W1; mv1_src src; int K; };
@@ -474,25 +484,48 @@
 }
 
 struct mv2_q4k_act { u32x4 a[4]; uint32_t bsw; float yd; };
-static __device__ __forceinline__ void mv2_q4k_dot(const u32x4 H, const u32x4 Q, const u32x4 P, const mv2_q4k_act & A, uint32_t sel, float & acc, float & accm) {
+struct mv2_q4k_w { u32x4 ql, qh, pl, ph; int sc0, sc1, mn0, mn1; float dx, dmin; };
+static __device__ __forceinline__ mv2_q4k_w mv2_q4k_unpack(const u32x4 H, const u32x4 Q, const u32x4 P, uint32_t sel) {
+    mv2_q4k_w w;
     const uint32_t s_lo = H[1] & 0x3f3f3f3fu, s_hi = (H[3] & 0x0f0f0f0fu) | ((H[1] >> 2) & 0x30303030u);
     const uint32_t m_lo = H[2] & 0x3f3f3f3fu, m_hi = ((H[3] >> 4) & 0x0f0f0f0fu) | ((H[2] >> 2) & 0x30303030u);
     const uint32_t sw = __builtin_amdgcn_perm(s_hi, s_lo, sel), mw = __builtin_amdgcn_perm(m_hi, m_lo, sel);
-    const int sc0 = sw & 0xff, sc1 = sw >> 8;
-    const int mn0 = mw & 0xff, mn1 = mw >> 8;
-    const float dx = h2f((uint16_t) (H[0] & 0xffff)), dmin = h2f((uint16_t) (H[0] >> 16));
+    w.sc0 = sw & 0xff; w.sc1 = sw >> 8;
+    w.mn0 = mw & 0xff; w.mn1 = mw >> 8;
+    w.dx = h2f((uint16_t) (H[0] & 0xffff)); w.dmin = h2f((uint16_t) (H[0] >> 16));
+#pragma unroll
+    for (int k = 0; k < 4; ++k) { w.ql[k] = Q[k] & 0x0f0f0f0fu; w.qh[k] = (Q[k] >> 4) & 0x0f0f0f0fu; w.pl[k] = P[k] & 0x0f0f0f0fu; w.ph[k] = (P[k] >> 4) & 0x0f0f0f0fu; }
+    return w;
+}
+static __device__ __forceinline__ void mv2_q4k_fin(const mv2_q4k_w & w, const mv2_q4k_act & A, float & acc, float & accm) {
     const int bs0 = (int) (int16_t) (A.bsw & 0xffff), bs1 = (int) (int16_t) (A.bsw >> 16);
     int dl = 0, dh = 0;
 #pragma unroll
     for (int k = 0; k < 4; ++k) {
-        dl = dot4(Q[k] & 0x0f0f0f0fu, A.a[0][k], dl); dh = dot4((Q[k] >> 4) & 0x0f0f0f0fu, A.a[2][k], dh);
-        dl = dot4(P[k] & 0x0f0f0f0fu, A.a[1][k], dl); dh = dot4((P[k] >> 4) & 0x0f0f0f0fu, A.a[3][k], dh);
-    }
-    const int isum = mad24(sc0, dl, mul24(sc1, dh));
-    const int msum = mad24(mn0, bs0, mul24(mn1, bs1));
-    acc  = fmaf(dx * A.yd, (float) isum, acc);
-    accm = fmaf(dmin * A.yd, (float) msum, accm);
-}
+        dl = dot4(w.ql[k], A.a[0][k], dl); dh = dot4(w.qh[k], A.a[2][k], dh);
+        dl = dot4(w.pl[k], A.a[1][k], dl); dh = dot4(w.ph[k], A.a[3][k], dh);
+    }
+    const int isum = mad24(w.sc0, dl, mul24(w.sc1, dh));
+    const int msum = mad24(w.mn0, bs0, mul24(w.mn1, bs1));
+    acc  = fmaf(w.dx * A.yd, (float) isum, acc);
+    accm = fmaf(w.dmin * A.yd, (float) msum, accm);
+}
+static __device__ __forceinline__ void mv2_q4k_dot(const u32x4 H, const u32x4 Q, const u32x4 P, const mv2_q4k_act & A, uint32_t sel, float & acc, float & accm) {
+    mv2_q4k_fin(mv2_q4k_unpack(H, Q, P, sel), A, acc, accm);
+}
+template <bool UNP> struct mv2_q4k_held;
+template <> struct mv2_q4k_held<true> {
+    mv2_q4k_w w;
+    __device__ __forceinline__ void set(const u32x4 H, const u32x4 Q, const u32x4 P, uint32_t sel) { w = mv2_q4k_unpack(H, Q, P, sel); }
+    __device__ __forceinline__ mv2_q4k_w get(uint32_t) const { return w; }
+    __device__ __forceinline__ void pin() { mv2_pin(w.ql); mv2_pin(w.qh); mv2_pin(w.pl); mv2_pin(w.ph); mv2_pin(w.sc0); mv2_pin(w.sc1); mv2_pin(w.mn0); mv2_pin(w.mn1); mv2_pin(w.dx); mv2_pin(w.dmin); }
+};
+template <> struct mv2_q4k_held<false> {
+    u32x4 H, Q, P;
+    __device__ __forceinline__ void set(const u32x4 H_, const u32x4 Q_, const u32x4 P_, uint32_t) { H = H_; Q = Q_; P = P_; }
+    __device__ __forceinline__ mv2_q4k_w get(uint32_t sel) const { return mv2_q4k_unpack(H, Q, P, sel); }
+    __device__ __forceinline__ void pin() { mv2_pin(H); mv2_pin(Q); mv2_pin(P); }
+};
 static __device__ __forceinline__ void mv2_q4k_act_load(const char * im, int nb, int ib, int q, mv2_q4k_act & A) {
     const char * la = im + ib * 272 + 64 * q;
 #pragma unroll
@@ -501,36 +534,43 @@
     A.yd  = *(const float *) (im + mv1_img_d(nb) + ib * 4);
 }
 static __device__ __forceinline__ uint32_t mv2_q4k_sel(int q) { return 0x0c0c0000u | (uint32_t) ((q < 2 ? 0 : 4) + 2 * (q & 1)) | ((uint32_t) ((q < 2 ? 0 : 4) + 2 * (q & 1) + 1) << 8); }
-template <int R, int NIT, int C, bool PAIR, int XS = 0>
-static __device__ __forceinline__ void mv2_consume_q4k(const char * im, const char * ringp, int K, int c, int ntask, char * dst, int row0, float resid, mv2_flags * F) {
+template <int R, int NIT, int C, bool PAIR, int XS = 0, bool PREP = (MV2_PREPARE != 0), class Gate>
+static __device__ __forceinline__ void mv2_consume_q4k(const char * im, const char * ringp, int K, int c, int ntask, char * dst, int row0, mv2_flags * F, Gate && gate) {
     typedef mv2_geo<2304, R, NIT, XS> geo;
     constexpr int SLOTB = geo::SLOTB, NS = geo::NS;
+    constexpr bool UNP = C <= 11;
     const int lane = threadIdx.x & 63, nb = K >> 8;
     int blk, q; mv2_lane_map(lane, blk, q);
     const uint32_t sel = mv2_q4k_sel(q);
-    mv2_q4k_act A[NIT];
-#pragma unroll
-    for (int it = 0; it < NIT; ++it) mv2_q4k_act_load(im, nb, it * 16 + blk, q, A[it]);
     const char * wl = ringp + blk * 144;
     uint32_t seen = 0;
+    auto prep = [&](int j, int k, int it, mv2_q4k_held<UNP> (&w)[R]) {
+        const int t = __builtin_amdgcn_readfirstlane(j * NIT + it);
+        mv2_wait_step(t, seen, F);
+        const char * p = wl + (t % NS) * SLOTB;
+        u32x4 H[R], Q[R], P[R];
+#pragma unroll
+        for (int r = 0; r < R; ++r) { H[r] = *(const u32x4 *) (p + r * 2304); Q[r] = *(const u32x4 *) (p + r * 2304 + 16 + 32 * q); P[r] = *(const u32x4 *) (p + r * 2304 + 32 + 32 * q); }
+        if (it == NIT - 1) { MV2_LGKM0(); mv2_poke(MV2_FLAG(F->consumed[c]), (uint32_t) (k + 1)); }
+#pragma unroll
+        for (int r = 0; r < R; ++r) w[r].set(H[r], Q[r], P[r], sel);
+    };
+    float resid = 0.0f;
+    int j = c, k = 0;
+    mv2_q4k_held<UNP> w0[NIT][R];
+    if constexpr (PREP) {
+        if (c >= ntask) return;
+#pragma unroll
+        for (int it = 0; it < NIT; ++it) { prep(c, 0, it, w0[it]);
+#pragma unroll
+            for (int r = 0; r < R; ++r) w0[it][r].pin(); }
+    }
+    resid = gate();
+    mv2_q4k_act A[NIT];
+#pragma unroll
+    for (int it = 0; it < NIT; ++it) mv2_q4k_act_load(im, nb, it * 16 + blk, q, A[it]);
     mv2_out o = { 0.0f, 0, 0 };
-    int k = 0;
-    for (int j = c; j < ntask; j += C, ++k) {
-        float acc[R], accm[R];
-#pragma unroll
-        for (int r = 0; r < R; ++r) { acc[r] = 0.0f; accm[r] = 0.0f; }
-#pragma unroll
-        for (int it = 0; it < NIT; ++it) {
-            const int t = __builtin_amdgcn_readfirstlane(j * NIT + it);
-            mv2_wait_step(t, seen, F);
-            const char * p = wl + (t % NS) * SLOTB;
-            u32x4 H[R], Q[R], P[R];
-#pragma unroll
-            for (int r = 0; r < R; ++r) { H[r] = *(const u32x4 *) (p + r * 2304); Q[r] = *(const u32x4 *) (p + r * 2304 + 16 + 32 * q); P[r] = *(const u32x4 *) (p + r * 2304 + 32 + 32 * q); }
-            if (it == NIT - 1) { MV2_LGKM0(); mv2_poke(MV2_FLAG(F->consumed[c]), (uint32_t) (k + 1)); }
-#pragma unroll
-            for (int r = 0; r < R; ++r) mv2_q4k_dot(H[r], Q[r], P[r], A[it], sel, acc[r], accm[r]);
-        }
+    auto done = [&](const float (&acc)[R], const float (&accm)[R]) {
         if (PAIR) {
             const float gsum = wave_sum_f32(acc[0] - accm[0]), usum = wave_sum_f32(acc[R - 1] - accm[R - 1]);
             if (lane == o.nres) o.res = mv1_silu(gsum) * usum;
@@ -539,65 +579,107 @@
             if (lane == o.nres) o.res = s;
         }
         if (++o.nres == 64) mv2_out_flush<C>(o, dst, row0, resid);
+    };
+    if constexpr (PREP) {
+        float acc[R], accm[R];
+#pragma unroll
+        for (int r = 0; r < R; ++r) { acc[r] = 0.0f; accm[r] = 0.0f; }
+#pragma unroll
+        for (int it = 0; it < NIT; ++it)
+#pragma unroll
+            for (int r = 0; r < R; ++r) mv2_q4k_fin(w0[it][r].get(sel), A[it], acc[r], accm[r]);
+        done(acc, accm);
+        j += C; k = 1;
+    }
+    for (; j < ntask; j += C, ++k) {
+        float acc[R], accm[R];
+#pragma unroll
+        for (int r = 0; r < R; ++r) { acc[r] = 0.0f; accm[r] = 0.0f; }
+#pragma unroll
+        for (int it = 0; it < NIT; ++it) {
+            mv2_q4k_held<UNP> w[R];
+            prep(j, k, it, w);
+#pragma unroll
+            for (int r = 0; r < R; ++r) mv2_q4k_fin(w[r].get(sel), A[it], acc[r], accm[r]);
+        }
+        done(acc, accm);
     }
     mv2_out_flush<C>(o, dst, row0, resid);
 }
 
-template <int NIT, int C, bool PAIR, int XS = 0>
-static __device__ __forceinline__ void mv2_consume_q4k_b(const char * im, const char * ringp, int K, int c, int ntask, char * dst, int G0, const char * rstg, bool has_resid, mv2_flags * F) {
+template <bool NIB, int NQ> struct mv2_q4kb_held {
+    u32x4 lo[NQ], hi[NIB ? NQ : 1];
+    uint32_t s_lo, s_hi, m_lo, m_hi; float dx, dmin;
+    __device__ __forceinline__ void set(const u32x4 H, const u32x4 (&Q)[NQ]) {
+        s_lo = H[1] & 0x3f3f3f3fu; s_hi = (H[3] & 0x0f0f0f0fu) | ((H[1] >> 2) & 0x30303030u);
+        m_lo = H[2] & 0x3f3f3f3fu; m_hi = ((H[3] >> 4) & 0x0f0f0f0fu) | ((H[2] >> 2) & 0x30303030u);
+        dx = h2f((uint16_t) (H[0] & 0xffff)); dmin = h2f((uint16_t) (H[0] >> 16));
+#pragma unroll
+        for (int e = 0; e < NQ; ++e) { if constexpr (NIB) { lo[e] = Q[e] & 0x0f0f0f0fu; hi[e] = (Q[e] >> 4) & 0x0f0f0f0fu; } else lo[e] = Q[e]; }
+    }
+    __device__ __forceinline__ uint32_t ql(int e, int i) const { return NIB ? lo[e][i] : lo[e][i] & 0x0f0f0f0fu; }
+    __device__ __forceinline__ uint32_t qh(int e, int i) const { return NIB ? hi[e][i] : (lo[e][i] >> 4) & 0x0f0f0f0fu; }
+    __device__ __forceinline__ void pin() {
+#pragma unroll
+        for (int e = 0; e < NQ; ++e) { mv2_pin(lo[e]); if constexpr (NIB) mv2_pin(hi[e]); }
+        mv2_pin(s_lo); mv2_pin(s_hi); mv2_pin(m_lo); mv2_pin(m_hi); mv2_pin(dx); mv2_pin(dmin);
+    }
+};
+template <int NIT, int C, bool PAIR, int XS = 0, bool PREP = (MV2_PREPARE != 0), class Gate>
+static __device__ __forceinline__ void mv2_consume_q4k_b(const char * im, const char * ringp, int K, int c, int ntask, char * dst, int G0, const char * rstg, bool has_resid, mv2_flags * F, Gate && gate) {
     constexpr int R = PAIR ? 2 : 1, GR = PAIR ? 2 : 4;
     typedef mv2_geo<2304, R, NIT, XS> geo;
     constexpr int SLOTB = geo::SLOTB, NS = geo::NS;
+    typedef mv2_q4kb_held<!PAIR, 8> held;
     const int lane = threadIdx.x & 63, nb = K >> 8;
     const int blk = lane & 15, r = PAIR ? lane >> 5 : lane >> 4, mat = PAIR ? (lane >> 4) & 1 : 0;
     const int ng = (ntask + GR - 1) / GR;
     uint32_t seen = 0;
-    int k = 0;
-    for (int g = c; g < ng; g += C, ++k) {
+    auto prep = [&](int g, int k, int it, held & w) {
         const int j = g * GR + r;
         const bool valid = j < ntask;
         const int jl = (g * GR + GR <= ntask ? g * GR + GR : ntask) - 1;
-        float accv = 0.0f, accm = 0.0f;
-#pragma unroll
-        for (int it = 0; it < NIT; ++it) {
-            mv2_wait_step(__builtin_amdgcn_readfirstlane(jl * NIT + it), seen, F);
-            const int t = (valid ? j : jl) * NIT + it;
-            const int b0 = __builtin_amdgcn_readfirstlane((g * GR * NIT + it) % NS);
-            int slot = b0 + (t - (g * GR * NIT + it));
-            if (slot >= NS) slot -= NS;
-            const char * p = ringp + slot * SLOTB + mat * 2304 + blk * 144;
-            const u32x4 H = *(const u32x4 *) p;
-            u32x4 Q[8];
-#pragma unroll
-            for (int e = 0; e < 8; ++e) Q[e] = *(const u32x4 *) (p + 16 + 16 * e);
-            const int ib = it * 16 + blk;
-            const char * la = im + ib * 272;
-            const u32x4 bsv = *(const u32x4 *) (im + mv1_img_bs(nb) + ib * 16);
-            const float yd = *(const float *) (im + mv1_img_d(nb) + ib * 4);
-            if (it == NIT - 1) { MV2_LGKM0(); mv2_poke(MV2_FLAG(F->consumed[c]), (uint32_t) (k + 1)); }
-            const uint32_t s_lo = H[1] & 0x3f3f3f3fu, s_hi = (H[3] & 0x0f0f0f0fu) | ((H[1] >> 2) & 0x30303030u);
-            const uint32_t m_lo = H[2] & 0x3f3f3f3fu, m_hi = ((H[3] >> 4) & 0x0f0f0f0fu) | ((H[2] >> 2) & 0x30303030u);
-            int isum = 0, msum = 0;
-#pragma unroll
-            for (int jg = 0; jg < 4; ++jg) {
-                const u32x4 a0 = *(const u32x4 *) (la + 64 * jg), a1 = *(const u32x4 *) (la + 64 * jg + 16), a2 = *(const u32x4 *) (la + 64 * jg + 32), a3 = *(const u32x4 *) (la + 64 * jg + 48);
-                int dl = 0, dh = 0;
-#pragma unroll
-                for (int e = 0; e < 4; ++e) {
-                    dl = dot4(Q[2 * jg][e] & 0x0f0f0f0fu, a0[e], dl); dh = dot4((Q[2 * jg][e] >> 4) & 0x0f0f0f0fu, a2[e], dh);
-                    dl = dot4(Q[2 * jg + 1][e] & 0x0f0f0f0fu, a1[e], dl); dh = dot4((Q[2 * jg + 1][e] >> 4) & 0x0f0f0f0fu, a3[e], dh);
-                }
-                const uint32_t sw = jg < 2 ? s_lo : s_hi, mw = jg < 2 ? m_lo : m_hi;
-                const int sh = 16 * (jg & 1);
-                const int sc0 = (int) ((sw >> sh) & 0xffu), sc1 = (int) ((sw >> (sh + 8)) & 0xffu), mn0 = (int) ((mw >> sh) & 0xffu), mn1 = (int) ((mw >> (sh + 8)) & 0xffu);
-                const uint32_t bw = bsv[jg];
-                isum = mad24(sc0, dl, mad24(sc1, dh, isum));
-                msum = mad24(mn0, (int) (int16_t) (bw & 0xffff), mad24(mn1, (int) (int16_t) (bw >> 16), msum));
+        mv2_wait_step(__builtin_amdgcn_readfirstlane(jl * NIT + it), seen, F);
+        const int t = (valid ? j : jl) * NIT + it;
+        const int b0 = __builtin_amdgcn_readfirstlane((g * GR * NIT + it) % NS);
+        int slot = b0 + (t - (g * GR * NIT + it));
+        if (slot >= NS) slot -= NS;
+        const char * p = ringp + slot * SLOTB + mat * 2304 + blk * 144;
+        const u32x4 H = *(const u32x4 *) p;
+        u32x4 Q[8];
+#pragma unroll
+        for (int e = 0; e < 8; ++e) Q[e] = *(const u32x4 *) (p + 16 + 16 * e);
+        if (it == NIT - 1) { MV2_LGKM0(); mv2_poke(MV2_FLAG(F->consumed[c]), (uint32_t) (k + 1)); }
+        w.set(H, Q);
+    };
+    auto fin = [&](int it, const held & w, float & accv, float & accm) {
+        const int ib = it * 16 + blk;
+        const char * la = im + ib * 272;
+        const u32x4 bsv = *(const u32x4 *) (im + mv1_img_bs(nb) + ib * 16);
+        const float yd = *(const float *) (im + mv1_img_d(nb) + ib * 4);
+        int isum = 0, msum = 0;
+#pragma unroll
+        for (int jg = 0; jg < 4; ++jg) {
+            const u32x4 a0 = *(const u32x4 *) (la + 64 * jg), a1 = *(const u32x4 *) (la + 64 * jg + 16), a2 = *(const u32x4 *) (la + 64 * jg + 32), a3 = *(const u32x4 *) (la + 64 * jg + 48);
+            int dl = 0, dh = 0;
+#pragma unroll
+            for (int e = 0; e < 4; ++e) {
+                dl = dot4(w.ql(2 * jg, e), a0[e], dl); dh = dot4(w.qh(2 * jg, e), a2[e], dh);
+                dl = dot4(w.ql(2 * jg + 1, e), a1[e], dl); dh = dot4(w.qh(2 * jg + 1, e), a3[e], dh);
             }
-            const float dx = h2f((uint16_t) (H[0] & 0xffff)), dmin = h2f((uint16_t) (H[0] >> 16));
-            accv = fmaf(dx * yd, (float) isum, accv);
-            accm = fmaf(dmin * yd, (float) msum, accm);
-        }
+            const uint32_t sw = jg < 2 ? w.s_lo : w.s_hi, mw = jg < 2 ? w.m_lo : w.m_hi;
+            const int sh = 16 * (jg & 1);
+            const int sc0 = (int) ((sw >> sh) & 0xffu), sc1 = (int) ((sw >> (sh + 8)) & 0xffu), mn0 = (int) ((mw >> sh) & 0xffu), mn1 = (int) ((mw >> (sh + 8)) & 0xffu);
+            const uint32_t bw = bsv[jg];
+            isum = mad24(sc0, dl, mad24(sc1, dh, isum));
+            msum = mad24(mn0, (int) (int16_t) (bw & 0xffff), mad24(mn1, (int) (int16_t) (bw >> 16), msum));
+        }
+        accv = fmaf(w.dx * yd, (float) isum, accv);
+        accm = fmaf(w.dmin * yd, (float) msum, accm);
+    };
+    auto done = [&](int g, float accv, float accm) {
+        const int j = g * GR + r;
+        const bool valid = j < ntask;
         float v = accv - accm;
         v += __uint_as_float(mv2_dpp_row<0xB1>(__float_as_uint(v))); v += __uint_as_float(mv2_dpp_row<0x4E>(__float_as_uint(v)));
         v += __uint_as_float(mv2_dpp_row<0x141>(__float_as_uint(v))); v += __uint_as_float(mv2_dpp_row<0x140>(__float_as_uint(v)));
@@ -607,11 +689,38 @@
         } else {
             if (valid && blk == 0) *(float *) (dst + (size_t) (G0 + j) * 4) = v + (has_resid ? *(const float *) (rstg + j * 4) : 0.0f);
         }
-    }
-}
-
-template <int NIT, int C, int XS = 0>
-static __device__ __forceinline__ void mv2_consume_q4k_h(const char * im, const char * ringp, int K, int c, int ntask, char * dst, int G0, const char * rstg, bool has_resid, mv2_flags * F) {
+    };
+    int g = c, k = 0;
+    if constexpr (PREP) {
+        if (c >= ng) return;
+        held w0[NIT];
+#pragma unroll
+        for (int it = 0; it < NIT; ++it) { prep(c, 0, it, w0[it]); w0[it].pin(); }
+        gate();
+        float accv = 0.0f, accm = 0.0f;
+#pragma unroll
+        for (int it = 0; it < NIT; ++it) fin(it, w0[it], accv, accm);
+        done(c, accv, accm);
+        g += C; k = 1;
+    } else gate();
+    for (; g < ng; g += C, ++k) {
+        float accv = 0.0f, accm = 0.0f;
+#pragma unroll
+        for (int it = 0; it < NIT; ++it) { held w; prep(g, k, it, w); fin(it, w, accv, accm); }
+        done(g, accv, accm);
+    }
+}
+
+struct mv2_q4kh_held {
+    u32x4 lo[4], hi[4]; uint32_t sw, mw; float dx, dmin;
+    __device__ __forceinline__ void pin() {
+#pragma unroll
+        for (int e = 0; e < 4; ++e) { mv2_pin(lo[e]); mv2_pin(hi[e]); }
+        mv2_pin(sw); mv2_pin(mw); mv2_pin(dx); mv2_pin(dmin);
+    }
+};
+template <int NIT, int C, int XS = 0, bool PREP = (MV2_PREPARE != 0), class Gate>
+static __device__ __forceinline__ void mv2_consume_q4k_h(const char * im, const char * ringp, int K, int c, int ntask, char * dst, int G0, const char * rstg, bool has_resid, mv2_flags * F, Gate && gate) {
     constexpr int GR = 2;
     typedef mv2_geo<2304, 1, NIT, XS> geo;
     constexpr int SLOTB = geo::SLOTB, NS = geo::NS;
@@ -619,58 +728,80 @@
     const int blk = lane & 15, h = (lane >> 4) & 1, r = lane >> 5;
     const int ng = (ntask + GR - 1) / GR;
     uint32_t seen = 0;
-    int k = 0;
-    for (int g = c; g < ng; g += C, ++k) {
+    auto prep = [&](int g, int k, int it, mv2_q4kh_held & w) {
         const int j = g * GR + r;
         const bool valid = j < ntask;
         const int jl = (g * GR + GR <= ntask ? g * GR + GR : ntask) - 1;
-        float accv = 0.0f, accm = 0.0f;
-#pragma unroll
-        for (int it = 0; it < NIT; ++it) {
-            mv2_wait_step(__builtin_amdgcn_readfirstlane(jl * NIT + it), seen, F);
-            const int t = (valid ? j : jl) * NIT + it;
-            const int b0 = __builtin_amdgcn_readfirstlane((g * GR * NIT + it) % NS);
-            int slot = b0 + (t - (g * GR * NIT + it));
-            if (slot >= NS) slot -= NS;
-            const char * p = ringp + slot * SLOTB + blk * 144;
-            const u32x4 H = *(const u32x4 *) p;
-            u32x4 Q[4];
-#pragma unroll
-            for (int e = 0; e < 4; ++e) Q[e] = *(const u32x4 *) (p + 16 + 64 * h + 16 * e);
-            const int ib = it * 16 + blk;
-            const char * la = im + ib * 272 + 128 * h;
-            u32x4 a[8];
-#pragma unroll
-            for (int e = 0; e < 8; ++e) a[e] = *(const u32x4 *) (la + 16 * e);
-            const u32x2 bsv = *(const u32x2 *) (im + mv1_img_bs(nb) + ib * 16 + 8 * h);
-            const float yd = *(const float *) (im + mv1_img_d(nb) + ib * 4);
-            if (it == NIT - 1) { MV2_LGKM0(); mv2_poke(MV2_FLAG(F->consumed[c]), (uint32_t) (k + 1)); }
-            const uint32_t sw = h ? ((H[3] & 0x0f0f0f0fu) | ((H[1] >> 2) & 0x30303030u)) : (H[1] & 0x3f3f3f3fu);
-            const uint32_t mw = h ? (((H[3] >> 4) & 0x0f0f0f0fu) | ((H[2] >> 2) & 0x30303030u)) : (H[2] & 0x3f3f3f3fu);
-            int isum = 0, msum = 0;
-#pragma unroll
-            for (int tj = 0; tj < 2; ++tj) {
-                int dl = 0, dh = 0;
-#pragma unroll
-                for (int e = 0; e < 4; ++e) {
-                    dl = dot4(Q[2 * tj][e] & 0x0f0f0f0fu, a[4 * tj][e], dl);         dh = dot4((Q[2 * tj][e] >> 4) & 0x0f0f0f0fu, a[4 * tj + 2][e], dh);
-                    dl = dot4(Q[2 * tj + 1][e] & 0x0f0f0f0fu, a[4 * tj + 1][e], dl); dh = dot4((Q[2 * tj + 1][e] >> 4) & 0x0f0f0f0fu, a[4 * tj + 3][e], dh);
-                }
-                const int sh = 16 * tj;
-                const int sc0 = (int) ((sw >> sh) & 0xffu), sc1 = (int) ((sw >> (sh + 8)) & 0xffu), mn0 = (int) ((mw >> sh) & 0xffu), mn1 = (int) ((mw >> (sh + 8)) & 0xffu);
-                const uint32_t bw = bsv[tj];
-                isum = mad24(sc0, dl, mad24(sc1, dh, isum));
-                msum = mad24(mn0, (int) (int16_t) (bw & 0xffff), mad24(mn1, (int) (int16_t) (bw >> 16), msum));
+        mv2_wait_step(__builtin_amdgcn_readfirstlane(jl * NIT + it), seen, F);
+        const int t = (valid ? j : jl) * NIT + it;
+        const int b0 = __builtin_amdgcn_readfirstlane((g * GR * NIT + it) % NS);
+        int slot = b0 + (t - (g * GR * NIT + it));
+        if (slot >= NS) slot -= NS;
+        const char * p = ringp + slot * SLOTB + blk * 144;
+        const u32x4 H = *(const u32x4 *) p;
+        u32x4 Q[4];
+#pragma unroll
+        for (int e = 0; e < 4; ++e) Q[e] = *(const u32x4 *) (p + 16 + 64 * h + 16 * e);
+        if (it == NIT - 1) { MV2_LGKM0(); mv2_poke(MV2_FLAG(F->consumed[c]), (uint32_t) (k + 1)); }
+        w.sw = h ? ((H[3] & 0x0f0f0f0fu) | ((H[1] >> 2) & 0x30303030u)) : (H[1] & 0x3f3f3f3fu);
+        w.mw = h ? (((H[3] >> 4) & 0x0f0f0f0fu) | ((H[2] >> 2) & 0x30303030u)) : (H[2] & 0x3f3f3f3fu);
+        w.dx = h2f((uint16_t) (H[0] & 0xffff)); w.dmin = h2f((uint16_t) (H[0] >> 16));
+#pragma unroll
+        for (int e = 0; e < 4; ++e) { w.lo[e] = Q[e] & 0x0f0f0f0fu; w.hi[e] = (Q[e] >> 4) & 0x0f0f0f0fu; }
+    };
+    auto fin = [&](int it, const mv2_q4kh_held & w, float & accv, float & accm) {
+        const int ib = it * 16 + blk;
+        const char * la = im + ib * 272 + 128 * h;
+        u32x4 a[8];
+#pragma unroll
+        for (int e = 0; e < 8; ++e) a[e] = *(const u32x4 *) (la + 16 * e);
+        const u32x2 bsv = *(const u32x2 *) (im + mv1_img_bs(nb) + ib * 16 + 8 * h);
+        const float yd = *(const float *) (im + mv1_img_d(nb) + ib * 4);
+        int isum = 0, msum = 0;
+#pragma unroll
+        for (int tj = 0; tj < 2; ++tj) {
+            int dl = 0, dh = 0;
+#pragma unroll
+            for (int e = 0; e < 4; ++e) {
+                dl = dot4(w.lo[2 * tj][e], a[4 * tj][e], dl);         dh = dot4(w.hi[2 * tj][e], a[4 * tj + 2][e], dh);
+                dl = dot4(w.lo[2 * tj + 1][e], a[4 * tj + 1][e], dl); dh = dot4(w.hi[2 * tj + 1][e], a[4 * tj + 3][e], dh);
             }
-            const float dx = h2f((uint16_t) (H[0] & 0xffff)), dmin = h2f((uint16_t) (H[0] >> 16));
-            accv = fmaf(dx * yd, (float) isum, accv);
-            accm = fmaf(dmin * yd, (float) msum, accm);
-        }
+            const int sh = 16 * tj;
+            const int sc0 = (int) ((w.sw >> sh) & 0xffu), sc1 = (int) ((w.sw >> (sh + 8)) & 0xffu), mn0 = (int) ((w.mw >> sh) & 0xffu), mn1 = (int) ((w.mw >> (sh + 8)) & 0xffu);
+            const uint32_t bw = bsv[tj];
+            isum = mad24(sc0, dl, mad24(sc1, dh, isum));
+            msum = mad24(mn0, (int) (int16_t) (bw & 0xffff), mad24(mn1, (int) (int16_t) (bw >> 16), msum));
+        }
+        accv = fmaf(w.dx * yd, (float) isum, accv);
+        accm = fmaf(w.dmin * yd, (float) msum, accm);
+    };
+    auto done = [&](int g, float accv, float accm) {
+        const int j = g * GR + r;
+        const bool valid = j < ntask;
         float v = accv - accm;
         v += __uint_as_float(mv2_dpp_row<0xB1>(__float_as_uint(v))); v += __uint_as_float(mv2_dpp_row<0x4E>(__float_as_uint(v)));
         v += __uint_as_float(mv2_dpp_row<0x141>(__float_as_uint(v))); v += __uint_as_float(mv2_dpp_row<0x140>(__float_as_uint(v)));
         { const auto sw2 = __builtin_amdgcn_permlane16_swap(__float_as_uint(v), __float_as_uint(v), false, false); v = __uint_as_float((uint32_t) sw2[0]) + __uint_as_float((uint32_t) sw2[1]); }
         if (valid && blk == 0 && h == 0) *(float *) (dst + (size_t) (G0 + j) * 4) = v + (has_resid ? *(const float *) (rstg + j * 4) : 0.0f);
+    };
+    int g = c, k = 0;
+    if constexpr (PREP) {
+        if (c >= ng) return;
+        mv2_q4kh_held w0[NIT];
+#pragma unroll
+        for (int it = 0; it < NIT; ++it) { prep(c, 0, it, w0[it]); w0[it].pin(); }
+        gate();
+        float accv = 0.0f, accm = 0.0f;
+#pragma unroll
+        for (int it = 0; it < NIT; ++it) fin(it, w0[it], accv, accm);
+        done(c, accv, accm);
+        g += C; k = 1;
+    } else gate();
+    for (; g < ng; g += C, ++k) {
+        float accv = 0.0f, accm = 0.0f;
+#pragma unroll
+        for (int it = 0; it < NIT; ++it) { mv2_q4kh_held w; prep(g, k, it, w); fin(it, w, accv, accm); }
+        done(g, accv, accm);
     }
 }
 
@@ -707,53 +838,99 @@
     Rg.sc[0] = __builtin_amdgcn_alignbit(d3[1], d3[0], L.sh); Rg.sc[1] = __builtin_amdgcn_alignbit(d3[2], d3[1], L.sh);
     Rg.dw = *(const uint16_t *) (p + 208);
 }
-static __device__ __forceinline__ float mv2_q6k_dot(const mv2_q6k_regs & Rg, const mv2_q6k_act & A, uint32_t sel, float acc) {
-    const uint32_t scw = __builtin_amdgcn_perm(Rg.sc[1], Rg.sc[0], sel);
+struct mv2_q6k_w { u32x4 v[4]; uint32_t scw; float d; };
+static __device__ __forceinline__ mv2_q6k_w mv2_q6k_unpack(const mv2_q6k_regs & Rg, uint32_t sel) {
+    mv2_q6k_w w;
+    w.scw = __builtin_amdgcn_perm(Rg.sc[1], Rg.sc[0], sel);
+#pragma unroll
+    for (int e = 0; e < 4; ++e) {
+        const uint32_t Aq = Rg.qla[e], Bq = Rg.qlb[e], Hq = Rg.qh[e];
+        w.v[0][e] = (Aq & 0x0f0f0f0fu)        | ((Hq << 4) & 0x30303030u);
+        w.v[1][e] = (Bq & 0x0f0f0f0fu)        | ((Hq << 2) & 0x30303030u);
+        w.v[2][e] = ((Aq >> 4) & 0x0f0f0f0fu) | (Hq & 0x30303030u);
+        w.v[3][e] = ((Bq >> 4) & 0x0f0f0f0fu) | ((Hq >> 2) & 0x30303030u);
+    }
+    w.d = h2f(Rg.dw);
+    return w;
+}
+static __device__ __forceinline__ float mv2_q6k_fin(const mv2_q6k_w & w, const mv2_q6k_act & A, float acc) {
     const int bs[4] = { (int) (int16_t) (A.bq[0] & 0xffff), (int) (int16_t) (A.bq[0] >> 16), (int) (int16_t) (A.bq[1] & 0xffff), (int) (int16_t) (A.bq[1] >> 16) };
     int d[4] = { 0, 0, 0, 0 };
 #pragma unroll
     for (int e = 0; e < 4; ++e) {
-        const uint32_t Aq = Rg.qla[e], Bq = Rg.qlb[e], Hq = Rg.qh[e];
-        d[0] = dot4((Aq & 0x0f0f0f0fu)        | ((Hq << 4) & 0x30303030u), A.a[0][e], d[0]);
-        d[1] = dot4((Bq & 0x0f0f0f0fu)        | ((Hq << 2) & 0x30303030u), A.a[1][e], d[1]);
-        d[2] = dot4(((Aq >> 4) & 0x0f0f0f0fu) | (Hq & 0x30303030u),        A.a[2][e], d[2]);
-        d[3] = dot4(((Bq >> 4) & 0x0f0f0f0fu) | ((Hq >> 2) & 0x30303030u), A.a[3][e], d[3]);
+        d[0] = dot4(w.v[0][e], A.a[0][e], d[0]);
+        d[1] = dot4(w.v[1][e], A.a[1][e], d[1]);
+        d[2] = dot4(w.v[2][e], A.a[2][e], d[2]);
+        d[3] = dot4(w.v[3][e], A.a[3][e], d[3]);
     }
     int isum = 0;
 #pragma unroll
     for (int m = 0; m < 4; ++m) {
-        const int scm = (int) (int8_t) ((scw >> (8 * m)) & 0xff);
+        const int scm = (int) (int8_t) ((w.scw >> (8 * m)) & 0xff);
         isum = mad24(scm, mad24(bs[m], -32, d[m]), isum);
     }
-    return fmaf(h2f(Rg.dw) * A.yd, (float) isum, acc);
-}
-template <int NIT, int C, int XS = 0>
-static __device__ __forceinline__ void mv2_consume_q6k(const char * im, const char * ringp, int K, int c, int ntask, char * dst, int row0, float resid, mv2_flags * F) {
+    return fmaf(w.d * A.yd, (float) isum, acc);
+}
+static __device__ __forceinline__ float mv2_q6k_dot(const mv2_q6k_regs & Rg, const mv2_q6k_act & A, uint32_t sel, float acc) { return mv2_q6k_fin(mv2_q6k_unpack(Rg, sel), A, acc); }
+template <bool UNP> struct mv2_q6k_held;
+template <> struct mv2_q6k_held<true> {
+    mv2_q6k_w w;
+    __device__ __forceinline__ void set(const mv2_q6k_regs & Rg, uint32_t sel) { w = mv2_q6k_unpack(Rg, sel); }
+    __device__ __forceinline__ mv2_q6k_w get(uint32_t) const { return w; }
+    __device__ __forceinline__ void pin() { mv2_pin(w.v[0]); mv2_pin(w.v[1]); mv2_pin(w.v[2]); mv2_pin(w.v[3]); mv2_pin(w.scw); mv2_pin(w.d); }
+};
+template <> struct mv2_q6k_held<false> {
+    mv2_q6k_regs Rg;
+    __device__ __forceinline__ void set(const mv2_q6k_regs & Rg_, uint32_t) { Rg = Rg_; }
+    __device__ __forceinline__ mv2_q6k_w get(uint32_t sel) const { return mv2_q6k_unpack(Rg, sel); }
+    __device__ __forceinline__ void pin() { mv2_pin(Rg.qla); mv2_pin(Rg.qlb); mv2_pin(Rg.qh); uint32_t a = Rg.sc[0], b = Rg.sc[1], d = Rg.dw; mv2_pin(a); mv2_pin(b); mv2_pin(d); Rg.sc[0] = a; Rg.sc[1] = b; Rg.dw = (uint16_t) d; }
+};
+template <int NIT, int C, int XS = 0, bool PREP = (MV2_PREPARE != 0), class Gate>
+static __device__ __forceinline__ void mv2_consume_q6k(const char * im, const char * ringp, int K, int c, int ntask, char * dst, int row0, mv2_flags * F, Gate && gate) {
     typedef mv2_geo<3360, 1, NIT, XS> geo;
     constexpr int SLOTB = geo::SLOTB, NS = geo::NS;
+    constexpr bool UNP = C <= 11;
     const int lane = threadIdx.x & 63, nb = K >> 8;
     const mv2_q6k_lane L = mv2_q6k_lane_of(lane);
-    mv2_q6k_act A[NIT];
-#pragma unroll
-    for (int it = 0; it < NIT; ++it) mv2_q6k_act_load(im, nb, it * 16 + L.blk, L, A[it]);
     const char * wl = ringp + L.blk * 210;
     uint32_t seen = 0;
+    auto prep = [&](int j, int k, int it, mv2_q6k_held<UNP> & w) {
+        const int t = __builtin_amdgcn_readfirstlane(j * NIT + it);
+        mv2_wait_step(t, seen, F);
+        mv2_q6k_regs Rg;
+        mv2_q6k_read(wl + (t % NS) * SLOTB, L, Rg);
+        if (it == NIT - 1) { MV2_LGKM0(); mv2_poke(MV2_FLAG(F->consumed[c]), (uint32_t) (k + 1)); }
+        w.set(Rg, L.sel);
+    };
+    int j = c, k = 0;
+    mv2_q6k_held<UNP> w0[NIT];
+    if constexpr (PREP) {
+        if (c >= ntask) return;
+#pragma unroll
+        for (int it = 0; it < NIT; ++it) { prep(c, 0, it, w0[it]); w0[it].pin(); }
+    }
+    const float resid = gate();
+    mv2_q6k_act A[NIT];
+#pragma unroll
+    for (int it = 0; it < NIT; ++it) mv2_q6k_act_load(im, nb, it * 16 + L.blk, L, A[it]);
     mv2_out o = { 0.0f, 0, 0 };
-    int k = 0;
-    for (int j = c; j < ntask; j += C, ++k) {
-        float acc = 0.0f;
-#pragma unroll
-        for (int it = 0; it < NIT; ++it) {
-            const int t = __builtin_amdgcn_readfirstlane(j * NIT + it);
-            mv2_wait_step(t, seen, F);
-            mv2_q6k_regs Rg;
-            mv2_q6k_read(wl + (t % NS) * SLOTB, L, Rg);
-            if (it == NIT - 1) { MV2_LGKM0(); mv2_poke(MV2_FLAG(F->consumed[c]), (uint32_t) (k + 1)); }
-            acc = mv2_q6k_dot(Rg, A[it], L.sel, acc);
-        }
+    auto done = [&](float acc) {
         const float s = wave_sum_f32(acc);
         if (lane == o.nres) o.res = s;
         if (++o.nres == 64) mv2_out_flush<C>(o, dst, row0, resid);
+    };
+    if constexpr (PREP) {
+        float acc = 0.0f;
+#pragma unroll
+        for (int it = 0; it < NIT; ++it) acc = mv2_q6k_fin(w0[it].get(L.sel), A[it], acc);
+        done(acc);
+        j += C; k = 1;
+    }
+    for (; j < ntask; j += C, ++k) {
+        float acc = 0.0f;
+#pragma unroll
+        for (int it = 0; it < NIT; ++it) { mv2_q6k_held<UNP> w; prep(j, k, it, w); acc = mv2_q6k_fin(w.get(L.sel), A[it], acc); }
+        done(acc);
     }
     mv2_out_flush<C>(o, dst, row0, resid);
 }
```

Result: no change. 614.9 tok/s, median of 6 (+0.2%).
